# davxy/ark-vrf

Measured on AMD Instinct MI355X. Metric: thin_vrf_batch_verifications_per_sec, higher is better.
Workload: dtype u32x8 (256-bit prime-field Montgomery, integer)

## Files before the change

### ark_vrf_amd/csrc/capi.hip

```cpp
#include "capi_internal.h"
#include "host_sha512.h"
#include "host_shake128.h"
#include "host_sha256.h"
#include "host_sha512_mb.h"
#include <condition_variable>
#include <deque>
#include <mutex>
#include <thread>
#include "proto_dev.h"
#include "vrf_batch.h"
#include "suite_dispatch.h"
#include <chrono>
#include <optional>
#include <stdlib.h>
#include <string.h>

using namespace avrf;

namespace avrf {
double now_us() {
  return std::chrono::duration<double, std::micro>(std::chrono::steady_clock::now().time_since_epoch()).count();
}
}

// ... 156 lines not shown
    HIP_TRY(c->d_misc.ensure(n * 64)); HIP_TRY(c->L->d_scalars.ensure(n * 32)); HIP_TRY(c->L->d_pre.ensure(n * sizeof(te_pre_raw)));
    HIP_TRY(hipMemcpyAsync(c->d_misc.p, bases_mont_xy, n * 64, hipMemcpyHostToDevice, c->stream));
    HIP_TRY(hipMemcpyAsync(c->L->d_scalars.p, scalars_mont, n * 32, hipMemcpyHostToDevice, c->stream));
    HIP_TRY(hipMemsetAsync(c->d_flags.p, 0, 4, c->stream));
    launch_pre_from_affine(c->suite, c->d_misc.as<uint8_t>(), n, c->L->d_pre.as<te_pre_raw>(), c->d_flags.as<uint32_t>(), 0, c->stream, 1);
    launch_scalars_from_mont(c->suite, c->L->d_scalars.as<uint32_t>(), n, c->d_flags.as<uint32_t>(), c->stream);
    HIP_TRY(hipMemcpyAsync(c->h_flags.p, c->d_flags.p, 4, hipMemcpyDeviceToHost, c->stream));
  }
  c->staged_kind = 0;
  if (int e = lane_msm(c, n, &r)) return e;
  if (n && *c->h_flags.as<uint32_t>()) return AVRF_INVALID_DATA;
  uint8_t canon[64];
  finish_point(c, r, canon);
  with_suite(c->suite, [&](auto tag) { using S = typename decltype(tag)::type; using Fq = HostField<typename S::Fq>;
    Fq::store_le(out_mont_xy, Fq::to_mont(Fq::load_le(canon))); Fq::store_le(out_mont_xy + 32, Fq::to_mont(Fq::load_le(canon + 32))); });
  return AVRF_OK;
}

int avrf_g1_msm(avrf_ctx *c, size_t n, const uint8_t *bases_xy, const uint8_t *scalars, uint8_t *out_xy) {
  if (!c || !out_xy || (n && (!bases_xy || !scalars))) return AVRF_ERR_BAD_ARG;
  if (ctx_busy(c)) return AVRF_ERR_BAD_ARG;
  HIP_TRY(hipSetDevice(c->device));
  const int curve = pairing_curve_of(c->suite);
  const size_t fqb = curve == 0 ? 48 : 32;
  for (size_t i = 0; i < n; i++) {
    H256 v; memcpy(v.l, scalars + 32 * i, 32);
    bool ok = curve == 0 ? !HostField<FqBandersnatch>::geq_p(v) : !HostField<FqBabyJubJub>::geq_p(v);
    if (!ok) return AVRF_INVALID_DATA;
  }
  c->staged_kind = 0;
  if (n) {
    HIP_TRY(c->d_misc.ensure(n * 2 * fqb)); HIP_TRY(c->L->d_scalars.ensure(n * 32)); HIP_TRY(c->L->d_pre.ensure(n * 2 * fqb));
    HIP_TRY(hipMemcpyAsync(c->d_misc.p, bases_xy, n * 2 * fqb, hipMemcpyHostToDevice, c->stream));
    HIP_TRY(hipMemcpyAsync(c->L->d_scalars.p, scalars, n * 32, hipMemcpyHostToDevice, c->stream));
    HIP_TRY(hipMemsetAsync(c->d_flags.p, 0, 4, c->stream));
    launch_g1_bases(curve, c->d_misc.as<uint8_t>(), n, c->L->d_pre.as<uint32_t>(), c->d_flags.as<uint32_t>(), c->stream);
    HIP_TRY(hipMemcpyAsync(c->h_flags.p, c->d_flags.p, 4, hipMemcpyDeviceToHost, c->stream));
  }
  if (int e = guarded([&] { return msm_g1_device(curve, c->L->d_pre.as<uint32_t>(), c->L->d_scalars.as<uint32_t>(), n, c->L->ws, c->stream, out_xy) ? (int)AVRF_ERR_BAD_ARG : 0; })) return e;
  if (n && *c->h_flags.as<uint32_t>()) return AVRF_INVALID_DATA;
  return AVRF_OK;
}


}
namespace avrf {
static bool suite_host_weights(int suite) { return with_suite(suite, [&](auto tag) { using S = typename decltype(tag)::type; return (bool)S::HOST_WEIGHTS; }); }
int ctx_stage(avrf_ctx *c, int kind, size_t n, const uint8_t *sks, const uint8_t *pks_xy, const uint8_t *ios_xy,
              const uint32_t *io_counts, const uint8_t *ads, const uint32_t *ad_lens, const uint8_t *proofs, bool wait) {
  if (!c || c->run_phase) return AVRF_ERR_BAD_ARG;
  if (n && (!io_counts || !ad_lens)) return AVRF_ERR_BAD_ARG;
  if (n > 0x0fffffffULL) return AVRF_ERR_BAD_ARG;
  HIP_TRY(hipSetDevice(c->device));
  c->staged_kind = 0; c->n = n; c->tot_io = 0; c->n_terms = 0; c->stage_gen++; c->wire_pending = false;
  if (n == 0) { c->staged_kind = kind; return AVRF_OK; }
  HIP_TRY(c->h_io.ensure((n + 1) * 8));
  uint32_t *io_off = c->h_io.as<uint32_t>(), *ad_off = io_off + (n + 1);
  uint64_t a = 0, b = 0;
  for (size_t j = 0; j < n; j++) { io_off[j] = (uint32_t)a; ad_off[j] = (uint32_t)b; a += io_counts[j]; b += ad_lens[j]; }
  if (a > 0x1fffffffULL || b > 0x7fffffffULL) return AVRF_ERR_BAD_ARG;
  if ((a && !ios_xy) || (b && !ads)) return AVRF_ERR_BAD_ARG;
  io_off[n] = (uint32_t)a; ad_off[n] = (uint32_t)b;
  c->tot_io = (size_t)a;
  HIP_TRY(c->d_io_off.ensure((n + 1) * 4)); HIP_TRY(c->d_ad_off.ensure((n + 1) * 4));
  HIP_TRY(c->d_ios.ensure(a * 128 + 16)); HIP_TRY(c->d_ads.ensure(b + 16));
  HIP_TRY(hipMemcpyAsync(c->d_io_off.p, io_off, (n + 1) * 4, hipMemcpyHostToDevice, c->stream));
  HIP_TRY(hipMemcpyAsync(c->d_ad_off.p, ad_off, (n + 1) * 4, hipMemcpyHostToDevice, c->stream));
  if (a) HIP_TRY(hipMemcpyAsync(c->d_ios.p, ios_xy, a * 128, hipMemcpyHostToDevice, c->stream));
  if (b) HIP_TRY(hipMemcpyAsync(c->d_ads.p, ads, b, hipMemcpyHostToDevice, c->stream));
  const size_t psz = kind == 1 ? 96 : kind == 3 ? 48 : 256;
  if (pks_xy) { HIP_TRY(c->d_pks.ensure(n * 64)); HIP_TRY(hipMemcpyAsync(c->d_pks.p, pks_xy, n * 64, hipMemcpyHostToDevice, c->stream)); }
  if (sks) { HIP_TRY(c->d_sks.ensure(n * 32)); HIP_TRY(hipMemcpyAsync(c->d_sks.p, sks, n * 32, hipMemcpyHostToDevice, c->stream)); }
  if (proofs) {
    HIP_TRY(c->d_proofs.ensure(n * psz)); HIP_TRY(hipMemcpyAsync(c->d_proofs.p, proofs, n * psz, hipMemcpyHostToDevice, c->stream));
    if (kind == 3) { HIP_TRY(hipStreamSynchronize(c->stream)); c->staged_kind = kind; return AVRF_OK; }
    if (suite_host_weights(c->suite)) {
      const size_t rsz = kind == 1 ? 32 : 64, roff = kind == 1 ? 64 : 192;
      c->h_resp.resize(n * rsz);
      for (size_t j = 0; j < n; j++) memcpy(&c->h_resp[rsz * j], proofs + psz * j + roff, rsz);
    }
    c->n_terms = kind == 1 ? 2 * n + 2 * c->tot_io + 1 : 5 * n + 2;
    HIP_TRY(c->d_c.ensure(n * 16)); HIP_TRY(c->h_c.ensure(n * 16));
    HIP_TRY(c->d_z.ensure(kind == 1 ? c->tot_io * 16 + 16 : n * 128));
    if (c->lane_owner) { HIP_TRY(c->L->d_scalars.ensure(c->n_terms * 32)); HIP_TRY(c->L->d_pre.ensure(c->n_terms * sizeof(te_pre_raw))); HIP_TRY(c->L->d_gpart.ensure(((n + 127) / 128) * 64 + 64)); }
  }
  if (wait) HIP_TRY(hipStreamSynchronize(c->stream));
  c->staged_kind = kind;
  return AVRF_OK;
}
int ctx_stage_wire(avrf_ctx *c, int kind, size_t n, const uint8_t *pks, const uint8_t *ios, const uint32_t *io_counts, const uint8_t *ads,
                   const uint32_t *ad_lens, const uint8_t *proofs, int validate, bool wait) {
  if (!c || c->run_phase || (kind != 1 && kind != 2)) return AVRF_ERR_BAD_ARG;
  if (n && (!io_counts || !ad_lens || !proofs || (kind == 1 && !pks))) return AVRF_ERR_BAD_ARG;
  if (n > 0x0fffffffULL) return AVRF_ERR_BAD_ARG;
  HIP_TRY(hipSetDevice(c->device));
  c->staged_kind = 0; c->n = n; c->tot_io = 0; c->n_terms = 0; c->stage_gen++; c->wire_pending = false;
  if (n == 0) { c->staged_kind = kind; return AVRF_OK; }
  HIP_TRY(c->h_io.ensure((n + 1) * 8));
  uint32_t *io_off = c->h_io.as<uint32_t>(), *ad_off = io_off + (n + 1);
  uint64_t a = 0, b = 0;
  for (size_t j = 0; j < n; j++) { io_off[j] = (uint32_t)a; ad_off[j] = (uint32_t)b; a += io_counts[j]; b += ad_lens[j]; }
  if (a > 0x1fffffffULL || b > 0x7fffffffULL) return AVRF_ERR_BAD_ARG;
  if ((a && !ios) || (b && !ads)) return AVRF_ERR_BAD_ARG;
  io_off[n] = (uint32_t)a; ad_off[n] = (uint32_t)b;
  c->tot_io = (size_t)a;
  const size_t L = (size_t)point_len_of(c->suite), ppts = kind == 1 ? 1 : 3, tail = kind == 1 ? 32 : 64, plen = ppts * L + tail, psz = kind == 1 ? 96 : 256;
  const size_t w_pks = kind == 1 ? n * L : 0, w_ios = 2 * (size_t)a * L, w_pr = n * plen;
  HIP_TRY(c->d_io_off.ensure((n + 1) * 4)); HIP_TRY(c->d_ad_off.ensure((n + 1) * 4));
  HIP_TRY(c->d_ios.ensure(a * 128 + 16)); HIP_TRY(c->d_ads.ensure(b + 16)); HIP_TRY(c->d_proofs.ensure(n * psz));
  if (kind == 1) HIP_TRY(c->d_pks.ensure(n * 64));
  HIP_TRY(c->d_misc.ensure(w_pks + w_ios + w_pr + 64)); HIP_TRY(c->d_status.ensure(64));
  uint8_t *dw = c->d_misc.as<uint8_t>();
  HIP_TRY(hipMemcpyAsync(c->d_io_off.p, io_off, (n + 1) * 4, hipMemcpyHostToDevice, c->stream));
  HIP_TRY(hipMemcpyAsync(c->d_ad_off.p, ad_off, (n + 1) * 4, hipMemcpyHostToDevice, c->stream));
  if (b) HIP_TRY(hipMemcpyAsync(c->d_ads.p, ads, b, hipMemcpyHostToDevice, c->stream));
  if (w_pks) HIP_TRY(hipMemcpyAsync(dw, pks, w_pks, hipMemcpyHostToDevice, c->stream));
  if (w_ios) HIP_TRY(hipMemcpyAsync(dw + w_pks, ios, w_ios, hipMemcpyHostToDevice, c->stream));
  HIP_TRY(hipMemcpyAsync(dw + w_pks + w_ios, proofs, w_pr, hipMemcpyHostToDevice, c->stream));
  uint32_t *d_flag = c->d_status.as<uint32_t>(), *h_flag = c->h_flags.as<uint32_t>() + 2;
  HIP_TRY(hipMemsetAsync(d_flag, 0, 4, c->stream));
  if (kind == 1) AVRF_SINGLE(c->suite, decompress_strided(dw, (uint32_t)L, (uint32_t)n, c->d_pks.as<uint8_t>(), 64, validate, d_flag, c->stream));
  AVRF_SINGLE(c->suite, decompress_strided(dw + w_pks, (uint32_t)L, (uint32_t)(2 * a), c->d_ios.as<uint8_t>(), 64, validate, d_flag, c->stream));
  const uint8_t *dpr = dw + w_pks + w_ios;
  for (size_t p = 0; p < ppts; p++)
    AVRF_SINGLE(c->suite, decompress_strided(dpr + L * p, (uint32_t)plen, (uint32_t)n, c->d_proofs.as<uint8_t>() + 64 * p, (uint32_t)psz, validate, d_flag, c->stream));
  HIP_TRY(hipMemcpy2DAsync(c->d_proofs.as<uint8_t>() + 64 * ppts, psz, dpr + L * ppts, plen, tail, n, hipMemcpyDeviceToDevice, c->stream));
  HIP_TRY(hipMemcpyAsync(h_flag, d_flag, 4, hipMemcpyDeviceToHost, c->stream));
  if (suite_host_weights(c->suite)) {
    const size_t rsz = kind == 1 ? 32 : 64, roff = ppts * L;
    c->h_resp.resize(n * rsz);
    for (size_t j = 0; j < n; j++) memcpy(&c->h_resp[rsz * j], proofs + plen * j + roff, rsz);
  }
  c->n_terms = kind == 1 ? 2 * n + 2 * c->tot_io + 1 : 5 * n + 2;
  HIP_TRY(c->d_c.ensure(n * 16)); HIP_TRY(c->h_c.ensure(n * 16));
  HIP_TRY(c->d_z.ensure(kind == 1 ? c->tot_io * 16 + 16 : n * 128));
  if (c->lane_owner) { HIP_TRY(c->L->d_scalars.ensure(c->n_terms * 32)); HIP_TRY(c->L->d_pre.ensure(c->n_terms * sizeof(te_pre_raw))); HIP_TRY(c->L->d_gpart.ensure(((n + 127) / 128) * 64 + 64)); }
  if (!wait) { c->wire_pending = true; c->staged_kind = kind; return AVRF_OK; }
  HIP_TRY(hipStreamSynchronize(c->stream)); HIP_TRY(hipGetLastError());
  if (*h_flag) return AVRF_INVALID_DATA;
  c->staged_kind = kind;
  return AVRF_OK;
}
}
extern "C" {
int avrf_thin_batch_stage_wire(avrf_ctx *c, size_t n, const uint8_t *pks, const uint8_t *ios, const uint32_t *io_counts, const uint8_t *ads,
                               const uint32_t *ad_lens, const uint8_t *proofs, int validate) {
  if (!c || ctx_busy(c)) return AVRF_ERR_BAD_ARG;
  return avrf::ctx_stage_wire(c, 1, n, pks, ios, io_counts, ads, ad_lens, proofs, validate, true);
}
int avrf_pedersen_batch_stage_wire(avrf_ctx *c, size_t n, const uint8_t *ios, const uint32_t *io_counts, const uint8_t *ads,
                                   const uint32_t *ad_lens, const uint8_t *proofs, int validate) {
  if (!c || ctx_busy(c)) return AVRF_ERR_BAD_ARG;
  return avrf::ctx_stage_wire(c, 2, n, nullptr, ios, io_counts, ads, ad_lens, proofs, validate, true);
}

int avrf_thin_batch_stage(avrf_ctx *c, size_t n, const uint8_t *pks_xy, const uint8_t *ios_xy, const uint32_t *io_counts,
                          const uint8_t *ads, const uint32_t *ad_lens, const uint8_t *proofs) {
  if (n && (!pks_xy || !proofs)) return AVRF_ERR_BAD_ARG;
  return ctx_stage(c, 1, n, nullptr, pks_xy, ios_xy, io_counts, ads, ad_lens, proofs, true);
}
int avrf_pedersen_batch_stage(avrf_ctx *c, size_t n, const uint8_t *ios_xy, const uint32_t *io_counts,
                              const uint8_t *ads, const uint32_t *ad_lens, const uint8_t *proofs) {
  if (n && !proofs) return AVRF_ERR_BAD_ARG;
  return ctx_stage(c, 2, n, nullptr, nullptr, ios_xy, io_counts, ads, ad_lens, proofs, true);
}

static void weight_digest_scalar(WeightJob &j) {
  HostSha512 h;
  if (j.msg) { h.update(j.msg, j.msg_len); h.final(j.digest); return; }
  h.update(j.prefix, j.prefix_len);
  uint8_t rec[96]; memset(rec, 0, sizeof rec);
  for (size_t k = 0; k < j.n; k++) { memcpy(rec, j.c16 + 16 * k, 16); memcpy(rec + 32, j.resp + j.rsz * k, j.rsz); h.update(rec, 32 + j.rsz); }
  h.final(j.digest);
}
namespace {
class WeightHashService {
 public:
  static WeightHashService &get() { static WeightHashService s; return s; }
  bool enabled() const { return !workers_.empty(); }
  void run(WeightJob &job) {
    Item it{&job, false};
    std::unique_lock<std::mutex> lk(m_);
    q_.push_back(&it);
    cv_work_.notify_one();
    cv_done_.wait(lk, [&] { return it.done; });
  }
 private:
  struct Item { WeightJob *job; bool done; };
  WeightHashService() {
    int n = 0;
    if (const char *e = getenv("AVRF_HASH_THREADS")) n = atoi(e);
    if (n < 0) n = 0; if (n > 16) n = 16;
    if (!sha512_mb_available()) n = 0;
    for (int i = 0; i < n; i++) workers_.emplace_back([this] { loop(); });
  }
  ~WeightHashService() {
    { std::lock_guard<std::mutex> lk(m_); stop_ = true; }
    cv_work_.notify_all();
    for (auto &t : workers_) t.join();
  }
  void loop() {
    for (;;) {
      Item *take[8]; int cnt = 0;
      {
        std::unique_lock<std::mutex> lk(m_);
        cv_work_.wait(lk, [&] { return stop_ || !q_.empty(); });
        if (stop_) return;
        if (q_.size() == 1) cv_work_.wait_for(lk, std::chrono::microseconds(40), [&] { return stop_ || q_.size() >= 2; });
        if (stop_) return;
        while (cnt < 8 && !q_.empty()) { take[cnt++] = q_.front(); q_.pop_front(); }
      }
      if (cnt == 1) weight_digest_scalar(*take[0]->job);
      else if (cnt > 1) { WeightJob *jobs[8]; for (int i = 0; i < cnt; i++) jobs[i] = take[i]->job; sha512_weights_x8(jobs, cnt); }
      { std::lock_guard<std::mutex> lk(m_); for (int i = 0; i < cnt; i++) take[i]->done = true; }
      cv_done_.notify_all();
    }
  }
  std::mutex m_; std::condition_variable cv_work_, cv_done_; std::deque<Item *> q_; std::vector<std::thread> workers_; bool stop_ = false;
};
// ... 20 lines not shown
  BatchDev b = batch_of(c);
  HIP_TRY(hipMemsetAsync(c->d_flags.p, 0, 4, c->stream));
  validate_staged(c, kind, nullptr);
  const int host_stream = host_stream_kind(c->suite);
  const size_t recsz = kind == 1 ? 64 : 96;
  uint8_t prefix[64]; const size_t pl = batch_prefix(c->suite, prefix);
  if (!host_stream) {
    HIP_TRY(c->d_rec.ensure(n * recsz)); HIP_TRY(c->h_msg.ensure(pl + n * recsz));
    b.records = c->d_rec.as<uint8_t>();
  }
  if (kind == 1) AVRF_BATCH(c->suite, thin_prepare(b, c->d_c.as<uint32_t>(), c->d_z.as<uint32_t>(), c->d_flags.as<uint32_t>(), c->stream));
  else AVRF_BATCH(c->suite, ped_prepare(b, c->d_c.as<uint32_t>(), c->d_z.as<uint8_t>(), c->d_flags.as<uint32_t>(), c->stream));
  if (!host_stream) {
    memcpy(c->h_msg.p, prefix, pl);
    HIP_TRY(hipMemcpyAsync(c->h_msg.as<uint8_t>() + pl, c->d_rec.p, n * recsz, hipMemcpyDeviceToHost, c->stream));
    c->h_msg_len = pl + n * recsz;
  } else HIP_TRY(hipMemcpyAsync(c->h_c.p, c->d_c.p, n * 16, hipMemcpyDeviceToHost, c->stream));
  HIP_TRY(hipMemcpyAsync(c->h_flags.p, c->d_flags.p, 4, hipMemcpyDeviceToHost, c->stream));
  c->run_begin_us = now_us() - c->run_t0;
  c->run_phase = 1;
  return AVRF_OK;
}

int batch_collect(avrf_ctx *c, int kind) {
  if (!c || c->staged_kind != kind || c->run_phase != 1) return AVRF_ERR_BAD_ARG;
  if (c->n && *c->h_flags.as<uint32_t>()) { c->run_phase = 0; return AVRF_INVALID_DATA; }
  if (c->wire_pending) {
    c->wire_pending = false;
    if (c->n && c->h_flags.as<uint32_t>()[2]) { c->run_phase = 0; c->staged_kind = 0; return AVRF_INVALID_DATA; }
  }
  return AVRF_OK;
}

int batch_seed(avrf_ctx *c, int kind, uint8_t digest[64]) {
  const size_t n = c->n;
  memset(digest, 0, 64);
  if (!n) return AVRF_OK;
  const int host_stream = host_stream_kind(c->suite);
  if (host_stream) {
    const uint8_t tag = DS_BATCH_VERIFY;
    const uint8_t *cs = c->h_c.as<uint8_t>();
    const size_t rsz = kind == 1 ? 32 : 64, wsz = kind == 1 ? 16 : 32;
    uint8_t rec[96]; memset(rec, 0, sizeof rec);
    c->h_weights.resize(n * wsz);
    auto run = [&](auto &h) {
      with_suite(c->suite, [&](auto tag_) { using S = typename decltype(tag_)::type; h.update(S::SUITE_ID, S::SUITE_ID_LEN); });
      h.update(&tag, 1);
      for (size_t j = 0; j < n; j++) { memcpy(rec, cs + 16 * j, 16); memcpy(rec + 32, &c->h_resp[rsz * j], rsz); h.update(rec, 32 + rsz); }
      h.squeeze_copy(c->h_weights.data(), n * wsz);
    };
    if (host_stream == 1) { HostShake128 h; run(h); } else { HostSha256 h; run(h); }
    return AVRF_OK;
  }
  WeightJob job; job.prefix = nullptr; job.prefix_len = 0; job.c16 = nullptr; job.resp = nullptr; job.n = n; job.rsz = 0;
  job.msg = c->h_msg.as<uint8_t>(); job.msg_len = c->h_msg_len;
  WeightHashService &svc = WeightHashService::get();
  if (svc.enabled()) svc.run(job); else weight_digest_scalar(job);
  memcpy(digest, job.digest, 64);
  return AVRF_OK;
}

int batch_launch(avrf_ctx *c, int kind, const uint8_t digest[64]) {
  if (!c || c->staged_kind != kind || c->run_phase != 1) return AVRF_ERR_BAD_ARG;
  if (c->n == 0) { c->run_phase = 2; return AVRF_OK; }
  c->run_phase = 0;
  HIP_TRY(hipSetDevice(c->device));
  const size_t n = c->n;
  BatchDev b = batch_of(c);
  if (c->unit_weights) {
    c->h_weights.assign(n * 16, 0);
    for (size_t j = 0; j < n; j++) c->h_weights[16 * j] = 1;
    HIP_TRY(c->d_weights.ensure(n * 16));
    HIP_TRY(hipMemcpyAsync(c->d_weights.p, c->h_weights.data(), n * 16, hipMemcpyHostToDevice, c->stream));
    b.weights = c->d_weights.as<uint8_t>();
  } else if (!host_stream_kind(c->suite)) b.records = c->d_rec.as<uint8_t>();
  else {
    const size_t wsz = kind == 1 ? 16 : 32;
    HIP_TRY(c->d_weights.ensure(n * wsz));
    HIP_TRY(hipMemcpyAsync(c->d_weights.p, c->h_weights.data(), n * wsz, hipMemcpyHostToDevice, c->stream));
    b.weights = c->d_weights.as<uint8_t>();
  }
  Seed64 seed;
  for (int i = 0; i < 8; i++) { uint64_t v; memcpy(&v, digest + 8 * i, 8); seed.w[i] = __builtin_bswap64(v); }
  HIP_TRY(c->L->d_scalars.ensure(c->n_terms * 32)); HIP_TRY(c->L->d_pre.ensure(c->n_terms * sizeof(te_pre_raw))); HIP_TRY(c->L->d_gpart.ensure(((n + 127) / 128) * 64 + 64));
  const double t2 = now_us();
  if (kind == 1) AVRF_BATCH(c->suite, thin_terms(b, seed, 0, c->d_c.as<uint32_t>(), c->d_z.as<uint32_t>(), c->L->d_scalars.as<uint32_t>(),
                                                 c->L->d_pre.as<te_pre_raw>(), c->L->d_gpart.as<uint32_t>(), (uint32_t)c->n_terms, c->stream));
  else AVRF_BATCH(c->suite, ped_terms(b, seed, 0, c->d_c.as<uint32_t>(), c->d_z.as<uint8_t>(), c->L->d_scalars.as<uint32_t>(),
                                      c->L->d_pre.as<te_pre_raw>(), c->L->d_gpart.as<uint32_t>(), (uint32_t)c->n_terms, c->stream));
  const double t3 = now_us();
  if (int e = guarded([&] { return msm_te_enqueue(c->suite, c->L->d_pre.as<te_pre_raw>(), c->L->d_scalars.as<uint32_t>(), c->n_terms, c->L->ws, c->chain(), c->stream) ? (int)AVRF_ERR_BAD_ARG : 0; })) return e;
  c->timing[3] = t3 - t2;
  c->run_msm_us = now_us() - t3;
  c->run_phase = 2;
  return AVRF_OK;
}

int batch_end(avrf_ctx *c, int kind) {
  if (!c || c->staged_kind != kind || c->run_phase != 2) return AVRF_ERR_BAD_ARG;
  c->run_phase = 0;
  if (c->n == 0) return AVRF_OK;
  HIP_TRY(hipSetDevice(c->device));
  const double t3 = now_us();
  HostExt r;
  if (int e = guarded([&] { return msm_te_finish(c->suite, c->L->ws, c->chain(), c->stream, &r) ? (int)AVRF_ERR_BAD_ARG : 0; })) return e;
  double t4 = now_us();
  int st = point_is_identity(c, r) ? AVRF_OK : AVRF_VERIFICATION_FAILURE;
  double t5 = now_us();
  c->timing[4] = c->run_msm_us + (t4 - t3); c->timing[5] = t5 - t4;
  c->timing[0] = c->timing[1] + c->timing[2] + c->timing[3] + c->timing[4] + c->timing[5];
  return st;
}
}
extern "C" {

static int batch_hash(avrf_ctx *c, int kind) {
  if (!c || c->staged_kind != kind || c->run_phase != 1) return AVRF_ERR_BAD_ARG;
  if (c->n == 0) { c->run_phase = 2; return AVRF_OK; }
  HIP_TRY(hipSetDevice(c->device));
  const double tw = now_us();
  if (hipStreamSynchronize(c->stream) != hipSuccess) { c->run_phase = 0; (void)hipGetLastError(); return AVRF_ERR_NO_DEVICE; }
  const double t1 = now_us();
  if (int e = batch_collect(c, kind)) return e;
  uint8_t digest[64];
  if (int e = batch_seed(c, kind, digest)) { c->run_phase = 0; return e; }
  const double t2 = now_us();
  c->timing[1] = c->run_begin_us + (t1 - tw); c->timing[2] = t2 - t1;
  return batch_launch(c, kind, digest);
}

static int batch_run(avrf_ctx *c, int kind) {
  if (int e = batch_begin(c, kind)) return e;
  if (int e = batch_hash(c, kind)) return e;
  return batch_end(c, kind);
}

int avrf_thin_batch_run(avrf_ctx *c) { return batch_run(c, 1); }
int avrf_pedersen_batch_run(avrf_ctx *c) { return batch_run(c, 2); }
static int run_call(avrf_ctx *c, int (*phase)(avrf_ctx *, int)) {
  if (!c) return AVRF_ERR_BAD_ARG;
  if (!c->staged_kind) {
    if (c->run_phase) { (void)hipSetDevice(c->device); (void)hipStreamSynchronize(c->stream); c->run_phase = 0; c->chain().disarm(); }
    return AVRF_ERR_BAD_ARG;
  }
  return phase(c, c->staged_kind);
}
int avrf_batch_run_begin(avrf_ctx *c) { return run_call(c, batch_begin); }
int avrf_batch_run_hash(avrf_ctx *c) { return run_call(c, batch_hash); }
int avrf_batch_run_end(avrf_ctx *c) { return run_call(c, batch_end); }

int avrf_thin_batch_verify(avrf_ctx *c, size_t n, const uint8_t *pks_xy, const uint8_t *ios_xy, const uint32_t *io_counts,
                           const uint8_t *ads, const uint32_t *ad_lens, const uint8_t *proofs) {
  int st = avrf_thin_batch_stage(c, n, pks_xy, ios_xy, io_counts, ads, ad_lens, proofs);
  return st ? st : avrf_thin_batch_run(c);
}
int avrf_pedersen_batch_verify(avrf_ctx *c, size_t n, const uint8_t *ios_xy, const uint32_t *io_counts,
                               const uint8_t *ads, const uint32_t *ad_lens, const uint8_t *proofs) {
  int st = avrf_pedersen_batch_stage(c, n, ios_xy, io_counts, ads, ad_lens, proofs);
  return st ? st : avrf_pedersen_batch_run(c);
}


int avrf_batch_weight_seed(int suite, int pedersen, size_t n, const uint8_t *c16, const uint8_t *resp, uint8_t seed_out[64]) {
  if (suite < 0 || suite >= AVRF_N_SUITES || !seed_out || (n && (!c16 || !resp))) return AVRF_ERR_BAD_ARG;
  if (with_suite(suite, [&](auto tag) { using S = typename decltype(tag)::type; return (bool)S::HOST_WEIGHTS; })) return AVRF_ERR_BAD_ARG;
  HostSha512 h;
  with_suite(suite, [&](auto tag) { using S = typename decltype(tag)::type; h.update(S::SUITE_ID, S::SUITE_ID_LEN); });
  const uint8_t tag = DS_BATCH_VERIFY; h.update(&tag, 1);
  const size_t rsz = pedersen ? 64 : 32;
  uint8_t rec[96]; memset(rec, 0, sizeof rec);
  for (size_t j = 0; j < n; j++) { memcpy(rec, c16 + 16 * j, 16); memcpy(rec + 32, resp + rsz * j, rsz); h.update(rec, 32 + rsz); }
  h.final(seed_out);
  return AVRF_OK;
}

int avrf_batch_weight_seeds_x8(int suite, int pedersen, int count, const size_t *n, const uint8_t *const *c16, const uint8_t *const *resp, uint8_t *seeds_out) {
  if (suite < 0 || suite >= AVRF_N_SUITES || count < 1 || count > 8 || !n || !c16 || !resp || !seeds_out) return AVRF_ERR_BAD_ARG;
  if (with_suite(suite, [&](auto tag) { using S = typename decltype(tag)::type; return (bool)S::HOST_WEIGHTS; })) return AVRF_ERR_BAD_ARG;
  if (!sha512_mb_available()) return AVRF_ERR_NO_DEVICE;
  uint8_t prefix[64]; size_t pl = 0;
  with_suite(suite, [&](auto tag) { using S = typename decltype(tag)::type; memcpy(prefix, S::SUITE_ID, S::SUITE_ID_LEN); pl = S::SUITE_ID_LEN; });
  prefix[pl++] = DS_BATCH_VERIFY;
  WeightJob jobs[8]; WeightJob *pj[8];
  for (int i = 0; i < count; i++) {
    if (n[i] && (!c16[i] || !resp[i])) return AVRF_ERR_BAD_ARG;
    jobs[i].prefix = prefix; jobs[i].prefix_len = pl; jobs[i].c16 = c16[i]; jobs[i].resp = resp[i]; jobs[i].n = n[i]; jobs[i].rsz = pedersen ? 64 : 32; pj[i] = &jobs[i];
  }
  sha512_weights_x8(pj, count);
  for (int i = 0; i < count; i++) memcpy(seeds_out + 64 * i, jobs[i].digest, 64);
  return AVRF_OK;
}

int avrf_sha512_x8(int count, const uint8_t *const *msgs, const size_t *lens, uint8_t *digests_out) {
  if (count < 1 || count > 8 || !msgs || !lens || !digests_out) return AVRF_ERR_BAD_ARG;
  if (!sha512_mb_available()) return AVRF_ERR_NO_DEVICE;
  static const uint8_t empty = 0;
  WeightJob jobs[8]; WeightJob *pj[8];
  for (int i = 0; i < count; i++) {
    if (lens[i] && !msgs[i]) return AVRF_ERR_BAD_ARG;
    jobs[i].msg = lens[i] ? msgs[i] : &empty; jobs[i].msg_len = lens[i]; pj[i] = &jobs[i];
  }
  sha512_weights_x8(pj, count);
  for (int i = 0; i < count; i++) memcpy(digests_out + 64 * i, jobs[i].digest, 64);
  return AVRF_OK;
}

int avrf_sha512_x16(int count, const uint8_t *const *msgs, const size_t *lens, uint8_t *digests_out) {
  if (count < 1 || count > 16 || !msgs || !lens || !digests_out) return AVRF_ERR_BAD_ARG;
  if (!sha512_mb16_available()) return AVRF_ERR_NO_DEVICE;
  static const uint8_t empty = 0;
  WeightJob jobs[16]; WeightJob *pj[16];
  for (int i = 0; i < count; i++) {
    if (lens[i] && !msgs[i]) return AVRF_ERR_BAD_ARG;
    jobs[i].msg = lens[i] ? msgs[i] : &empty; jobs[i].msg_len = lens[i]; pj[i] = &jobs[i];
  }
  sha512_weights_x16(pj, count);
  for (int i = 0; i < count; i++) memcpy(digests_out + 64 * i, jobs[i].digest, 64);
  return AVRF_OK;
}

int avrf_thin_batch_challenges(avrf_ctx *c, uint8_t *c_out) {
  if (!c || c->staged_kind != 1 || (c->n && !c_out)) return AVRF_ERR_BAD_ARG;
  if (ctx_busy(c)) return AVRF_ERR_BAD_ARG;
  if (c->n == 0) return AVRF_OK;
  HIP_TRY(hipSetDevice(c->device));
// ... 113 lines not shown

static int sync_stream(avrf_ctx *c) {
  HIP_TRY(hipStreamSynchronize(c->stream)); HIP_TRY(hipGetLastError());
  return AVRF_OK;
}

static bool wave_shape(const avrf_ctx *c, size_t n, const uint32_t *io_counts) {
  if (!n || n > (size_t)AVRF_WAVE_ITEMS_MAX || c->tot_io != n) return false;
  static const bool off = getenv("AVRF_NO_WAVE_ITEMS") != nullptr;
  if (off) return false;
  for (size_t j = 0; j < n; j++) if (io_counts[j] != 1) return false;
  return true;
}

using Route = std::optional<int>;
static bool one_as_msm() { static const bool on = getenv("AVRF_NO_ONE_AS_MSM") == nullptr; return on; }

static Route prove_one_as_msm(avrf_ctx *c, bool have_pk, bool tiny, uint8_t *proofs_out) {
  if (c->tot_io >= 1000) return {};
  const size_t nt = 1 + c->tot_io, plen = tiny ? 48 : 96, sb = AVRF_SINGLE(c->suite, prove_state_bytes());
  HIP_TRY(c->h_c.ensure(64));
  if (!have_pk) { if (int fs = ensure_fixed(c)) return fs; }
  HIP_TRY(c->L->d_scalars.ensure(nt * 32)); HIP_TRY(c->L->d_pre.ensure(nt * sizeof(te_pre_raw))); HIP_TRY(c->d_misc.ensure(sb + 64)); HIP_TRY(c->d_out.ensure(plen));
  BatchDev b = batch_of(c);
  if (!have_pk) b.pks_xy = nullptr;
  uint8_t *d_state = c->d_misc.as<uint8_t>();
  AVRF_SINGLE(c->suite, thin_prove_begin(b, c->L->d_scalars.as<uint32_t>(), c->L->d_pre.as<te_pre_raw>(), d_state, c->stream, tiny));
  HostExt r;
  if (int e = lane_msm(c, nt, &r)) return e;
  uint8_t *rxy = c->h_c.as<uint8_t>();
  finish_point(c, r, rxy);
  HIP_TRY(hipMemcpyAsync(d_state + sb, rxy, 64, hipMemcpyHostToDevice, c->stream));
  AVRF_SINGLE(c->suite, thin_prove_end(b, d_state, d_state + sb, c->d_out.as<uint8_t>(), c->d_flags.as<uint32_t>(), c->stream, tiny));
  HIP_TRY(hipMemcpyAsync(proofs_out, c->d_out.p, plen, hipMemcpyDeviceToHost, c->stream));
  return read_flags(c);
}

static Route prove_ped_one_as_msm(avrf_ctx *c, bool have_pk, uint8_t *proofs_out, uint8_t *blindings_out) {
  if (c->tot_io > 1000) return {};
  if (!have_pk) { if (int fs = ensure_fixed(c)) return fs; }
  const size_t m = c->tot_io, nt = 2 + m, sb = AVRF_SINGLE(c->suite, ped_state_bytes()), wb = (m * 32 + 63) / 64 * 64 + 64;
  HIP_TRY(c->L->d_scalars.ensure(2 * nt * 32)); HIP_TRY(c->L->d_pre.ensure(nt * sizeof(te_pre_raw)));
  HIP_TRY(c->d_misc.ensure(sb + wb + 192 + 32)); HIP_TRY(c->d_out.ensure(256)); HIP_TRY(c->h_c.ensure(192));
  BatchDev b = batch_of(c);
  if (!have_pk) b.pks_xy = nullptr;
  uint8_t *d_state = c->d_misc.as<uint8_t>(), *d_pts = d_state + sb + wb, *d_blind = d_pts + 192;
  uint32_t *d_wts = reinterpret_cast<uint32_t *>(d_state + sb);
  uint32_t *d_sc = c->L->d_scalars.as<uint32_t>(); te_pre_raw *d_pre = c->L->d_pre.as<te_pre_raw>();
  AVRF_SINGLE(c->suite, ped_prove_begin(b, d_sc, d_pre, d_state, d_wts, c->stream));
  HostExt r[2];
  if (int e = lane_msm(c, 2, &r[0])) return e;
  uint8_t *pts = c->h_c.as<uint8_t>();
  finish_point(c, r[0], pts);
  HIP_TRY(hipMemcpyAsync(d_pts, pts, 64, hipMemcpyHostToDevice, c->stream));
  AVRF_SINGLE(c->suite, ped_prove_mid(b, d_sc, d_pre, d_state, d_wts, d_pts, c->stream));
  if (int e = lane_msm_vectors(c, nt, 2, r)) return e;
  finish_point(c, r[0], pts + 64); finish_point(c, r[1], pts + 128);
  HIP_TRY(hipMemcpyAsync(d_pts + 64, pts + 64, 128, hipMemcpyHostToDevice, c->stream));
  AVRF_SINGLE(c->suite, ped_prove_end(b, d_state, d_pts, c->d_out.as<uint8_t>(), blindings_out ? d_blind : nullptr, c->d_flags.as<uint32_t>(), c->stream));
  HIP_TRY(hipMemcpyAsync(proofs_out, c->d_out.p, 256, hipMemcpyDeviceToHost, c->stream));
  if (blindings_out) HIP_TRY(hipMemcpyAsync(blindings_out, d_blind, 32, hipMemcpyDeviceToHost, c->stream));
  return read_flags(c);
}

static Route verify_one_as_msm(avrf_ctx *c, int32_t *status_out) {
  if (!c->n_terms || c->n_terms > 2048) return {};
  uint8_t zero[64] = {0};
  c->unit_weights = true;
  int st = batch_begin(c, 1);
  if (st == AVRF_OK) st = batch_launch(c, 1, zero);
  if (st == AVRF_OK) st = batch_end(c, 1);
  c->unit_weights = false;
  if (st != AVRF_OK && st != AVRF_VERIFICATION_FAILURE) { c->run_phase = 0; return st; }
  status_out[0] = *c->h_flags.as<uint32_t>() ? AVRF_INVALID_DATA : st;
  return AVRF_OK;
}

static Route verify_ped_one_as_msm(avrf_ctx *c, int32_t *status_out) {
  if (!c->n_terms || c->n_terms > 2048) return {};
  int st = batch_begin(c, 2);
  c->run_phase = 0;
  if (st != AVRF_OK) return st;
  const size_t nt = c->n_terms;
  HIP_TRY(c->L->d_scalars.ensure(2 * nt * 32)); HIP_TRY(c->L->d_pre.ensure(nt * sizeof(te_pre_raw))); HIP_TRY(c->L->d_gpart.ensure(2 * 64 + 64));
  c->h_weights.assign(64, 0); c->h_weights[0] = 1; c->h_weights[32 + 16] = 1;
  HIP_TRY(c->d_weights.ensure(64));
  HIP_TRY(hipMemcpyAsync(c->d_weights.p, c->h_weights.data(), 64, hipMemcpyHostToDevice, c->stream));
  BatchDev b = batch_of(c);
  Seed64 seed; for (int i = 0; i < 8; i++) seed.w[i] = 0;
  for (int v = 0; v < 2; v++) {
    b.weights = c->d_weights.as<uint8_t>() + 32 * v;
    AVRF_BATCH(c->suite, ped_terms(b, seed, 0, c->d_c.as<uint32_t>(), c->d_z.as<uint8_t>(), c->L->d_scalars.as<uint32_t>() + (size_t)v * nt * 8,
                                   c->L->d_pre.as<te_pre_raw>(), c->L->d_gpart.as<uint32_t>(), (uint32_t)nt, c->stream));
  }
  HostExt r[2];
  if (int e = lane_msm_vectors(c, nt, 2, r)) return e;
  status_out[0] = *c->h_flags.as<uint32_t>() ? AVRF_INVALID_DATA : (point_is_identity(c, r[0]) && point_is_identity(c, r[1])) ? AVRF_OK : AVRF_VERIFICATION_FAILURE;
  return AVRF_OK;
}

struct ItemCall {
  int kind;
  bool prover;
  size_t psz;
  uint8_t *proofs_out;
  uint8_t *blindings_out;
  int32_t *status_out;
};

template <class One, class Wave, class Lane>
static int item_call(avrf_ctx *c, const ItemCall &k, size_t n, const uint8_t *sks, const uint8_t *pks_xy, const uint8_t *ios_xy,
                     const uint32_t *io_counts, const uint8_t *ads, const uint32_t *ad_lens, const uint8_t *proofs, One one, Wave wave, Lane lane) {
  int st = ctx_stage(c, k.kind, n, sks, pks_xy, ios_xy, io_counts, ads, ad_lens, proofs, k.kind == 3);
  if (st || !n) return st;
  if (k.prover) {
    c->staged_kind = 0;
    HIP_TRY(c->d_out.ensure(n * k.psz));
    if (k.kind == 2) HIP_TRY(c->d_misc.ensure(n * 32));
  } else HIP_TRY(c->d_status.ensure(n * 4));
  if (k.prover || k.kind == 3) HIP_TRY(hipMemsetAsync(c->d_flags.p, 0, 4, c->stream));
  auto finish = [&](bool wave_statuses) -> int {
    if (!k.prover) {
      validate_staged(c, k.kind, c->d_status.as<int32_t>());
      HIP_TRY(hipMemcpyAsync(k.status_out, c->d_status.p, n * 4, hipMemcpyDeviceToHost, c->stream));
      return sync_stream(c);
    }
    HIP_TRY(hipMemcpyAsync(k.proofs_out, c->d_out.p, n * k.psz, hipMemcpyDeviceToHost, c->stream));
    if (k.blindings_out) HIP_TRY(hipMemcpyAsync(k.blindings_out, c->d_misc.p, n * 32, hipMemcpyDeviceToHost, c->stream));
    if (wave_statuses) HIP_TRY(hipMemcpyAsync(c->h_c.p, c->d_status.p, n * 4, hipMemcpyDeviceToHost, c->stream));
    return read_flags(c);
  };
  auto routes = [&]() -> int {
    if (n == 1 && one_as_msm()) { if (Route r = one()) return *r; }
    if ((!k.prover || pks_xy) && wave_shape(c, n, io_counts)) {
      if (k.prover && k.kind == 2) { if (int fs = ensure_fixed(c)) return fs; }
      if (k.prover) { HIP_TRY(c->d_status.ensure(n * 4)); HIP_TRY(c->h_c.ensure(n * 4)); }
      if (wave(batch_of(c))) {
        const int ws = finish(true);
        if (ws < 0) return ws;
        const int32_t *h_status = k.prover ? c->h_c.as<int32_t>() : k.status_out;
        bool fallback = false;
        for (size_t j = 0; j < n; j++) fallback |= h_status[j] == AVRF_WAVE_FALLBACK;
        if (!fallback) return ws;
        if (k.prover) HIP_TRY(hipMemsetAsync(c->d_flags.p, 0, 4, c->stream));
      }
    }
    if (int e = per_item_chunks(c, !k.prover || pks_xy, lane)) return e;
    return finish(false);
  };
  const double t0 = now_us();
  st = routes();
  c->timing[0] = now_us() - t0;
  if (k.kind == 3 && st == AVRF_OK) c->staged_kind = 0;
  return st;
}

template <class F> static int pointwise(avrf_ctx *c, size_t n, bool args_ok, F body) {
  if (!c || (n && !args_ok) || ctx_busy(c)) return AVRF_ERR_BAD_ARG;
  if (!n) return AVRF_OK;
  if (n > 0x7fffffffULL) return AVRF_ERR_BAD_ARG;
  HIP_TRY(hipSetDevice(c->device));
  c->staged_kind = 0;
  return body();
}
extern "C" {

static int thin_or_tiny_prove(avrf_ctx *c, bool tiny, size_t n, const uint8_t *sks, const uint8_t *pks_xy, const uint8_t *ios_xy,
// ... 156 lines not shown
```

### ark_vrf_amd/csrc/capi_internal.h

```cpp
#pragma once
#include "../../include/avrf.h"
#include "host_te.h"
#include "msm.h"
#include <hip/hip_runtime.h>
#include <stdio.h>
#include <new>
#include <vector>

#define HIP_TRY(x) do { hipError_t e_ = (x); if (e_ != hipSuccess) { fprintf(stderr, "avrf: HIP error %s at %s:%d\n", hipGetErrorString(e_), __FILE__, __LINE__); return AVRF_ERR_NO_DEVICE; } } while (0)

namespace avrf {

template <bool PINNED> struct StageBuf : OwnedMem<PINNED> {
  hipError_t ensure(size_t bytes) {
    if (bytes <= this->cap && this->p) return hipSuccess;
    return this->reset(PINNED ? bytes + 256 : bytes + bytes / 8 + 256);
  }
};
using DevBuf = StageBuf<false>;
using PinBuf = StageBuf<true>;

template <class F> int guarded(F f) {
  try { return f(); }
  catch (const avrf::HipFailure &e) { fprintf(stderr, "avrf: HIP error %s at %s:%d\n", hipGetErrorString(e.err), e.file, e.line); return AVRF_ERR_NO_DEVICE; }
  catch (const std::bad_alloc &) { return AVRF_ERR_NO_DEVICE; }
}

struct LaneStream {
  hipStream_t stream = nullptr;
  LaneStream() = default;
  LaneStream(const LaneStream &) = delete;
  LaneStream &operator=(const LaneStream &) = delete;
  ~LaneStream() { if (stream) (void)hipStreamDestroy(stream); }
};
struct Lane : LaneStream {
  int queued = 0;
  MsmWorkspace ws;
  DevBuf d_scalars, d_pre, d_gpart;
};

}

struct avrf_ctx {
  int suite = 0, device = 0;
  hipStream_t stream = nullptr;
  avrf::Lane own; avrf::Lane *L = &own;
  avrf::MsmChain *pend = nullptr;
  avrf::MsmChain &chain() const { return pend ? *pend : L->ws.own; }
  bool lane_owner = true;
  int validate = 0;
  bool wire_pending = false;
  uint64_t stage_gen = 0, chal_gen = 0;
  int staged_kind = 0;
  size_t n = 0, tot_io = 0, n_terms = 0;
  avrf::DevBuf d_pks, d_ios, d_io_off, d_ads, d_ad_off, d_proofs, d_sks;
  std::vector<uint8_t> h_resp;
  avrf::DevBuf d_rec; avrf::PinBuf h_msg;
  size_t h_msg_len = 0;
  std::vector<uint8_t> h_weights; avrf::DevBuf d_weights;
  avrf::DevBuf d_c, d_z, d_flags, d_misc, d_out, d_status;
  avrf::DevBuf d_tabs;
  avrf::DevBuf d_fixed; bool fixed_ready = false;
  avrf::PinBuf h_c, h_flags, h_io;
  double timing[8] = {0, 0, 0, 0, 0, 0, 0, 0};
  int run_phase = 0;
  bool unit_weights = false;
  double run_t0 = 0, run_begin_us = 0, run_msm_us = 0;
  ~avrf_ctx() { (void)hipSetDevice(device); if (own.stream) (void)hipStreamSynchronize(own.stream); }
};

namespace avrf {
int ctx_create(int suite, int device, bool lane_owner, avrf_ctx **out);
int ctx_stage(avrf_ctx *c, int kind, size_t n, const uint8_t *sks, const uint8_t *pks_xy, const uint8_t *ios_xy, const uint32_t *io_counts,
              const uint8_t *ads, const uint32_t *ad_lens, const uint8_t *proofs, bool wait);
int ctx_stage_wire(avrf_ctx *c, int kind, size_t n, const uint8_t *pks, const uint8_t *ios, const uint32_t *io_counts, const uint8_t *ads,
                   const uint32_t *ad_lens, const uint8_t *proofs, int validate, bool wait);
int batch_begin(avrf_ctx *c, int kind);
int batch_collect(avrf_ctx *c, int kind);
bool batch_host_weights(const avrf_ctx *c);
int batch_seed(avrf_ctx *c, int kind, uint8_t digest[64]);
int batch_launch(avrf_ctx *c, int kind, const uint8_t digest[64]);
int batch_end(avrf_ctx *c, int kind);
double now_us();
}
```

### ark_vrf_amd/csrc/msm.h

```cpp
#pragma once
#include <hip/hip_runtime.h>
#include <stddef.h>
#include <stdint.h>
#include "host_te.h"

namespace avrf {

struct te_pre_raw { uint32_t w[24]; };
struct te_ext_raw { uint32_t w[32]; };

struct HipFailure { hipError_t err; const char *file; int line; };

template <bool PINNED> struct OwnedMem {
  void *p = nullptr; size_t cap = 0;
  OwnedMem() = default;
  explicit OwnedMem(size_t bytes) { ensure(bytes); }
  OwnedMem(const OwnedMem &) = delete;
  OwnedMem &operator=(const OwnedMem &) = delete;
  OwnedMem(OwnedMem &&o) noexcept : p(o.p), cap(o.cap) { o.p = nullptr; o.cap = 0; }
  OwnedMem &operator=(OwnedMem &&o) noexcept { if (this != &o) { (void)release(); p = o.p; cap = o.cap; o.p = nullptr; o.cap = 0; } return *this; }
  ~OwnedMem() { (void)release(); }
  hipError_t reset(size_t bytes) {
    if (hipError_t e = release()) return e;
    if (hipError_t e = PINNED ? hipHostMalloc(&p, bytes) : hipMalloc(&p, bytes)) { p = nullptr; return e; }
    cap = bytes;
    return hipSuccess;
  }
  void ensure(size_t bytes) { if (bytes > cap) if (hipError_t e = reset(bytes)) throw HipFailure{e, __FILE__, __LINE__}; }
  hipError_t release() { hipError_t e = !p ? hipSuccess : PINNED ? hipHostFree(p) : hipFree(p); p = nullptr; cap = 0; return e; }
  template <class T = uint32_t> T *as() const { return (T *)p; }
  explicit operator bool() const { return p != nullptr; }
};
using DevMem = OwnedMem<false>;
using PinMem = OwnedMem<true>;
struct DevEvent {
  hipEvent_t e = nullptr;
  DevEvent() = default;
  DevEvent(const DevEvent &) = delete;
  DevEvent &operator=(const DevEvent &) = delete;
  DevEvent(DevEvent &&o) noexcept : e(o.e) { o.e = nullptr; }
  DevEvent &operator=(DevEvent &&o) noexcept { if (this != &o) { destroy(); e = o.e; o.e = nullptr; } return *this; }
  ~DevEvent() { destroy(); }
  hipError_t create(unsigned flags = hipEventDefault) { destroy(); return hipEventCreateWithFlags(&e, flags); }
  void destroy() { if (e) (void)hipEventDestroy(e); e = nullptr; }
  operator hipEvent_t() const { return e; }
};

struct MsmPlan {
  int c;
  int nwin;
  int nb;
  int lpb;
};
MsmPlan msm_plan(size_t n, int scalar_bits);

struct MsmChain {
  PinMem bits_host, plan_host;
  DevEvent ev0, ev1;
  MsmPlan plan = {0, 0, 0, 0}; int ret = 0;
  int wsum_lg = 4;
  size_t n = 0;
  bool armed = false;
  void ensure(size_t bytes);
  void disarm() { armed = false; }
  void release() { *this = MsmChain(); }
};

struct MsmWorkspace {
  DevMem keys;
  DevMem sorted;
  DevMem hist;
  DevMem cnts;
  DevMem offsets;
  DevMem win_tot;
  DevMem lane_base;
  DevMem heavy;
  DevMem plan_dev;
  DevMem buckets;
  DevMem rc;
  DevMem part;
  DevMem bits;
  MsmChain own;
  bool owns(const MsmChain &rec) const { return &rec == &own; }
  double accum_ms_total = 0; uint64_t accum_launches = 0; float accum_ms_last = 0;
  MsmPlan last_plan = {0, 0, 0, 0};
  void ensure(size_t n, const MsmPlan &p, size_t acc_bytes, size_t batch, size_t lanes_max, size_t part_bytes = 0);
  void release() { *this = MsmWorkspace(); }
};

int msm_te_device(int suite, const te_pre_raw *d_pre, const uint32_t *d_scalars, size_t n,
                  MsmWorkspace &ws, hipStream_t stream, HostExt *out);
int msm_te_enqueue(int suite, const te_pre_raw *d_pre, const uint32_t *d_scalars, size_t n, MsmWorkspace &ws, MsmChain &rec, hipStream_t stream);
int msm_te_finish(int suite, MsmWorkspace &ws, MsmChain &rec, hipStream_t stream, HostExt *out);
int msm_te_small_vectors(int suite, const te_pre_raw *d_pre, const uint32_t *d_scalars, size_t n, size_t n_vectors, MsmWorkspace &ws, hipStream_t stream,
                         HostExt *out);
bool msm_te_pending_supported(int suite);

int msm_g1_device(int curve, const uint32_t *d_bases, const uint32_t *d_scalars, size_t n, MsmWorkspace &ws, hipStream_t stream, uint8_t *out_xy,
                  size_t batch = 1, size_t scalar_stride = 0);
void build_g1_table(int curve, const uint32_t *d_bases, size_t n, int c, int nwin, uint32_t *d_table, hipStream_t stream);
int msm_g1_fixed_device(int curve, const uint32_t *d_table, int table_c, size_t table_stride, const uint32_t *d_scalars, size_t n,
                        size_t scalar_stride, MsmWorkspace &ws, hipStream_t stream, uint8_t *out_xy, size_t batch,
                        const uint32_t *d_base_idx = nullptr, int scalars_mont = 0);
struct G1DirectTable {
  uint32_t *d = nullptr;
  int curve = 0, c = 0, rows = 0;
  size_t n = 0;
  uint64_t off[32] = {};
  uint32_t mult[32] = {};
  uint64_t points = 0, bytes = 0;
};
size_t g1_direct_table_shape(int curve, size_t n, int c, G1DirectTable *t);
void build_g1_direct_table(int curve, const uint32_t *d_bases, size_t n, int c, G1DirectTable *t, hipStream_t stream);
void free_g1_direct_table(G1DirectTable *t);
int msm_g1_direct_device(const G1DirectTable &t, const uint32_t *d_scalars, size_t n, size_t scalar_stride, MsmWorkspace &ws, hipStream_t stream,
                         uint8_t *out_xy, size_t batch, int scalars_mont = 0, const uint32_t *d_base_idx = nullptr);
void launch_g1_decompress(int curve, const uint8_t *d_comp, size_t n, uint8_t *d_out_xy, uint8_t *d_ok, hipStream_t stream);
void launch_g1_bases(int curve, const uint8_t *d_xy, size_t n, uint32_t *d_out, uint32_t *d_flag, hipStream_t stream);
void launch_g1_subgroup_check(int curve, const uint32_t *d_bases, size_t n, uint32_t *d_flag, hipStream_t stream, int32_t *d_rec_status = nullptr,
                              uint32_t ppr = 1);
void launch_g1_lincomb(int curve, const uint32_t *d_bases, const uint32_t *d_scalars, size_t n_items, uint32_t tpi, uint32_t split, uint32_t *d_out,
                       hipStream_t stream, bool glv_split_scalars = false);
void g1_glv_split_bls(uint64_t k[4]);

void launch_pre_from_affine(int suite, const uint8_t *d_xy, size_t n, te_pre_raw *d_pre, uint32_t *d_flag,
                            int check_curve, hipStream_t stream, int mont_in = 0);
void launch_scalars_from_mont(int suite, uint32_t *d_scalars, size_t n, uint32_t *d_flag, hipStream_t stream);

}
```

### ark_vrf_amd/csrc/msm.hip

```cpp
#include "msm.h"
#include "host_pool.h"
#include "curves.h"
#include "suite_dispatch.h"
#include "te_quad.h"
#include "host_g1.h"
#include <stdio.h>
#include <stdlib.h>
#include <string.h>
#include <mutex>
#include <vector>

namespace avrf {

#define HIP_CHECK(x) do { hipError_t e_ = (x); if (e_ != hipSuccess) throw HipFailure{e_, __FILE__, __LINE__}; } while (0)


template <class S>
__global__ void __launch_bounds__(256) k_pre_from_affine(const uint8_t *__restrict__ xy, uint32_t n, te_pre *__restrict__ out,
                                  uint32_t *__restrict__ flag, int check_curve, int mont_in) {
  using Fq = typename S::Fq;
  uint32_t i = blockIdx.x * blockDim.x + threadIdx.x;
  if (i >= n) return;
  fp x = fp_load_le(xy + 64 * (size_t)i), y = fp_load_le(xy + 64 * (size_t)i + 32);
  uint32_t f = 0;
  if (ge_p<Fq>(x) || ge_p<Fq>(y)) f |= 1;
  fp xm = mont_in ? x : fp_to_mont<Fq>(x), ym = mont_in ? y : fp_to_mont<Fq>(y);
  if (check_curve && !te_on_curve<S>(xm, ym)) f |= 2;
  store_pre(out + i, te_make_pre<S>(xm, ym));
  if (f) atomicOr(flag, f);
}

void launch_pre_from_affine(int suite, const uint8_t *d_xy, size_t n, te_pre_raw *d_pre, uint32_t *d_flag,
                            int check_curve, hipStream_t stream, int mont_in) {
  if (!n) return;
  dim3 g((unsigned)((n + 255) / 256)), b(256);
  with_suite(suite, [&](auto tag) { using S = typename decltype(tag)::type;
    hipLaunchKernelGGL(k_pre_from_affine<S>, g, b, 0, stream, d_xy, (uint32_t)n, (te_pre *)d_pre, d_flag, check_curve, mont_in); });
}
template <class S>
__global__ void __launch_bounds__(256) k_scalars_from_mont(uint32_t *__restrict__ sc, uint32_t n, uint32_t *__restrict__ flag) {
  using Fr = typename S::Fr;
  uint32_t i = blockIdx.x * blockDim.x + threadIdx.x;
  if (i >= n) return;
  fp k = load_fp(sc + 8 * (size_t)i);
  if (ge_p<Fr>(k)) atomicOr(flag, 4u);
  store_fp(sc + 8 * (size_t)i, fp_from_mont<Fr>(k));
}
void launch_scalars_from_mont(int suite, uint32_t *d_scalars, size_t n, uint32_t *d_flag, hipStream_t stream) {
  if (!n) return;
  with_suite(suite, [&](auto tag) { using S = typename decltype(tag)::type;
    hipLaunchKernelGGL(k_scalars_from_mont<S>, dim3((unsigned)((n + 255) / 256)), dim3(256), 0, stream, d_scalars, (uint32_t)n, d_flag); });
}


__global__ void __launch_bounds__(256) k_digits(const uint32_t *__restrict__ scalars, uint32_t n, uint32_t stride, int c, int nwin, uint16_t *__restrict__ keys, int mont) {
  uint32_t i = blockIdx.x * blockDim.x + threadIdx.x;
  if (i >= n) return;
  const uint32_t bat = blockIdx.y;
  keys += (size_t)bat * nwin * n;
  uint32_t s[9];
  const uint4 *p = reinterpret_cast<const uint4 *>(scalars + 8 * ((size_t)bat * stride + i));
  uint4 a = p[0], b = p[1];
  s[0] = a.x; s[1] = a.y; s[2] = a.z; s[3] = a.w; s[4] = b.x; s[5] = b.y; s[6] = b.z; s[7] = b.w; s[8] = 0;
  if (mont) {
    fp v;
#pragma unroll
    for (int k = 0; k < 8; k++) v.v[k] = s[k];
    v = mont == 1 ? fp_from_mont<FqBandersnatch>(v) : fp_from_mont<FqBabyJubJub>(v);
#pragma unroll
    for (int k = 0; k < 8; k++) s[k] = v.v[k];
  }
  const uint32_t nb = 1u << (c - 1), mask = (1u << c) - 1;
  uint32_t carry = 0;
  for (int w = 0; w < nwin; w++) {
    int bit = w * c;
    uint32_t v = 0;
    if (bit < 256) {
      int li = bit >> 5, sh = bit & 31;
      uint64_t two = (uint64_t)s[li] | ((uint64_t)s[li + 1] << 32);
      v = (uint32_t)(two >> sh) & mask;
    }
    v += carry;
    uint32_t key;
    if (v > nb) { key = ((1u << c) - v) | 0x8000u; carry = 1; }
    else { key = v; carry = 0; }
    keys[(size_t)w * n + i] = (uint16_t)key;
  }
}


__global__ void __launch_bounds__(256)
k_hist(const uint16_t *__restrict__ keys, uint32_t n, uint32_t tile_len, int c, uint32_t *__restrict__ H) {
  extern __shared__ uint32_t lds[];
  const uint32_t nb = 1u << (c - 1), tile = blockIdx.x, w = blockIdx.y, ntiles = gridDim.x;
  for (uint32_t b = threadIdx.x; b < nb; b += blockDim.x) lds[b] = 0;
  __syncthreads();
  uint32_t lo = tile * tile_len, hi = lo + tile_len; if (hi > n) hi = n;
  const uint16_t *kw = keys + (size_t)w * n;
  for (uint32_t i = lo + threadIdx.x; i < hi; i += blockDim.x) {
    uint32_t b = kw[i] & 0x7fffu;
    if (b) atomicAdd(&lds[b - 1], 1u);
  }
  __syncthreads();
  uint32_t *out = H + ((size_t)w * ntiles + tile) * nb;
  for (uint32_t b = threadIdx.x; b < nb; b += blockDim.x) out[b] = lds[b];
}

__global__ void __launch_bounds__(256)
k_scan_tiles(uint32_t *__restrict__ H, uint32_t ntiles, int c, uint32_t *__restrict__ cnts) {
  const uint32_t nb = 1u << (c - 1), w = blockIdx.y, b = blockIdx.x * 256 + threadIdx.x;
  if (b >= nb) return;
  uint32_t *Hb = H + (size_t)w * ntiles * nb + b;
  uint32_t run = 0, k = 0;
  for (; k + 8 <= ntiles; k += 8) {
    uint32_t v[8];
#pragma unroll
    for (int j = 0; j < 8; j++) v[j] = Hb[(size_t)(k + j) * nb];
#pragma unroll
    for (int j = 0; j < 8; j++) { Hb[(size_t)(k + j) * nb] = run; run += v[j]; }
  }
  for (; k < ntiles; k++) { const uint32_t v = Hb[(size_t)k * nb]; Hb[(size_t)k * nb] = run; run += v; }
  cnts[(size_t)w * nb + b] = run;
}
__global__ void __launch_bounds__(1024)
k_scan_offs(const uint32_t *__restrict__ cnts, uint32_t n, int c, uint32_t *__restrict__ offs, uint32_t *__restrict__ win_tot) {
  __shared__ uint32_t part[1024];
  const uint32_t nb = 1u << (c - 1), w = blockIdx.x, t = threadIdx.x;
  const uint32_t bpt = (nb + 1023) / 1024;
  uint32_t b0 = t * bpt, b1 = b0 + bpt; if (b1 > nb) b1 = nb; if (b0 > nb) b0 = nb;
  uint32_t sum = 0;
  for (uint32_t b = b0; b < b1; b++) sum += cnts[(size_t)w * nb + b];
  part[t] = sum;
  __syncthreads();
  for (uint32_t off = 1; off < 1024; off <<= 1) {
    uint32_t v = (t >= off) ? part[t - off] : 0;
    __syncthreads();
    part[t] += v;
    __syncthreads();
  }
  if (t == 1023) win_tot[w] = part[1023];
  uint32_t run = part[t] - sum + w * n;
  for (uint32_t b = b0; b < b1; b++) { offs[(size_t)w * nb + b] = run; run += cnts[(size_t)w * nb + b]; }
}

__global__ void __launch_bounds__(1024)
k_plan(const uint32_t *__restrict__ win_tot, uint32_t vwin, uint32_t lanes_target, uint32_t per_min, uint32_t *__restrict__ lane_base,
       uint32_t *__restrict__ plan) {
  __shared__ uint64_t red[1024];
  __shared__ uint32_t sc[1024];
  __shared__ uint32_t carry_s;
  const uint32_t t = threadIdx.x;
  uint64_t s = 0;
  for (uint32_t v = t; v < vwin; v += 1024) s += win_tot[v];
  red[t] = s;
  __syncthreads();
  for (uint32_t off = 512; off >= 1; off >>= 1) { if (t < off) red[t] += red[t + off]; __syncthreads(); }
  const uint64_t total = red[0];
  if (lanes_target > 8 * vwin) lanes_target -= vwin;
  uint64_t per64 = (total + lanes_target - 1) / lanes_target;
  if (per64 < per_min) per64 = per_min;
  const uint32_t per = (uint32_t)per64;
  if (t == 0) carry_s = 0;
  __syncthreads();
  for (uint32_t base = 0; base < vwin; base += 1024) {
    const uint32_t v = base + t;
    const uint32_t mine = v < vwin ? (win_tot[v] + per - 1) / per : 0;
    sc[t] = mine;
    __syncthreads();
    for (uint32_t off = 1; off < 1024; off <<= 1) {
      uint32_t x = (t >= off) ? sc[t - off] : 0;
      __syncthreads();
      sc[t] += x;
      __syncthreads();
    }
    if (v < vwin) lane_base[v] = carry_s + sc[t] - mine;
    __syncthreads();
    if (t == 1023) carry_s += sc[1023];
    __syncthreads();
  }
  if (t == 0) { lane_base[vwin] = carry_s; plan[0] = per; plan[1] = carry_s; plan[2] = 0; }
}

__global__ void __launch_bounds__(256)
k_scatter(const uint16_t *__restrict__ keys, uint32_t n, uint32_t tile_len, int c, const uint32_t *__restrict__ H,
          const uint32_t *__restrict__ offs, uint32_t *__restrict__ sorted, uint32_t remap_n, uint32_t remap_stride,
          const uint32_t *__restrict__ bidx, uint32_t ntiles, uint32_t vwin) {
  extern __shared__ uint32_t lds[];
  const uint32_t nb = 1u << (c - 1);
  const uint32_t xcd = blockIdx.x & 7u, k = blockIdx.x >> 3, tile = k % ntiles, w = xcd + 8u * (k / ntiles);
  if (w >= vwin) return;
  const uint32_t *Hin = H + ((size_t)w * ntiles + tile) * nb;
  for (uint32_t b = threadIdx.x; b < nb; b += blockDim.x) lds[b] = offs[(size_t)w * nb + b] + Hin[b];
  __syncthreads();
  uint32_t lo = tile * tile_len, hi = lo + tile_len; if (hi > n) hi = n;
  const uint16_t *kw = keys + (size_t)w * n;
  for (uint32_t i = lo + threadIdx.x; i < hi; i += blockDim.x) {
    uint32_t key = kw[i], b = key & 0x7fffu;
    if (b) {
      uint32_t pos = atomicAdd(&lds[b - 1], 1u);
      uint32_t idx = i;
      if (remap_n) {
        uint32_t j = i % remap_n;
        idx = (i / remap_n) * remap_stride + (bidx ? bidx[(size_t)w * remap_n + j] : j);
      }
      sorted[pos] = idx | ((key & 0x8000u) << 16);
    }
  }
}

template <class CV> __device__ __noinline__ void cv_add_nf(typename CV::acc_t *r, const typename CV::acc_t *a, const typename CV::acc_t *b) { *r = CV::add(*a, *b); }
template <class CV> __device__ __noinline__ void cv_dbl_nf(typename CV::acc_t *r, const typename CV::acc_t *a) { *r = CV::dbl(*a); }
template <class CV> AVRF_DI typename CV::acc_t cv_add(const typename CV::acc_t &a, const typename CV::acc_t &b) {
  if constexpr (CV::INLINE_REDUCE_OPS) return CV::add(a, b);
  else { typename CV::acc_t r; cv_add_nf<CV>(&r, &a, &b); return r; }
}
template <class CV> AVRF_DI typename CV::acc_t cv_dbl(const typename CV::acc_t &a) {
  if constexpr (CV::INLINE_REDUCE_OPS) return CV::dbl(a);
  else { typename CV::acc_t r; cv_dbl_nf<CV>(&r, &a); return r; }
}



template <class CV>
__global__ void __launch_bounds__(256, CV::MIN_WAVES)
k_accumulate(const uint32_t *__restrict__ bases, const uint32_t *__restrict__ sorted,
             const uint32_t *__restrict__ offs, const uint32_t *__restrict__ win_tot, const uint32_t *__restrict__ lane_base,
             const uint32_t *__restrict__ plan, uint32_t vwin, uint32_t nb, uint32_t n, uint32_t *__restrict__ part) {
  using AC = typename CV::accum;
  using acc_t = typename AC::acc_t; using base_t = typename CV::base_t;
  const uint32_t t = blockIdx.x * blockDim.x + threadIdx.x;
  const uint32_t per = plan[0];
  if (t >= plan[1]) return;
  uint32_t lo = 0, hi = vwin;
  while (hi - lo > 1) { uint32_t mid = (lo + hi) >> 1; if (lane_base[mid] <= t) lo = mid; else hi = mid; }
  const uint32_t v = lo;
  const uint32_t wbeg = v * n, wend = wbeg + win_tot[v];
  const uint32_t e0 = wbeg + (t - lane_base[v]) * per;
  uint32_t e1 = e0 + per; if (e1 > wend) e1 = wend;
  const uint32_t *ow = offs + (size_t)v * nb;
  lo = 0; hi = nb;
  while (hi - lo > 1) { uint32_t mid = (lo + hi) >> 1; if (ow[mid] <= e0) lo = mid; else hi = mid; }
  uint32_t b = lo;
  uint32_t nxt = (b + 1 < nb) ? ow[b + 1] : 0xffffffffu;
  const size_t slot0 = (size_t)t + (size_t)v * nb;
  acc_t acc;
  {
    extern __shared__ uint32_t acc_lds[];
    constexpr int BW = CV::BASE_WORDS, CH = BW / 4;
    uint32_t *wbuf = acc_lds + (threadIdx.x >> 6) * (2 * BW * 64);
    const uint32_t lane = threadIdx.x & 63;
    auto issue = [&](uint32_t ix, uint32_t slot) {
      const uint32_t *src = bases + (size_t)(ix & 0x7fffffffu) * BW;
#pragma unroll
      for (int c = 0; c < CH; c++)
        __builtin_amdgcn_global_load_lds((const __attribute__((address_space(1))) void *)(src + 4 * c),
                                         (__attribute__((address_space(3))) void *)(wbuf + slot * (BW * 64) + c * 256), 16, 0, 0);
    };
    auto fetch = [&](uint32_t slot) {
      uint32_t w[BW];
#pragma unroll
      for (int c = 0; c < CH; c++) {
        const uint4 v = *reinterpret_cast<const uint4 *>(wbuf + slot * (BW * 64) + c * 256 + lane * 4);
        w[4 * c] = v.x; w[4 * c + 1] = v.y; w[4 * c + 2] = v.z; w[4 * c + 3] = v.w;
      }
      return CV::base_from_words(w);
    };
    const uint32_t cnt = e1 - e0;
    if constexpr (!CV::PREFETCH) acc = AC::identity();
    uint32_t idx = cnt ? sorted[e0] : 0u;
    uint32_t idx1 = cnt > 1 ? sorted[e0 + 1] : 0u;
    if (cnt) issue(idx, 0);
    for (uint32_t k = 0; k < cnt; k++) {
      const uint32_t i = e0 + k, cidx = idx;
      asm volatile("s_waitcnt vmcnt(0) lgkmcnt(0)" ::: "memory");
      const base_t cur = fetch(k & 1);
      idx = idx1;
      if (k + 1 < cnt) issue(idx, (k + 1) & 1);
      if (k + 2 < cnt) idx1 = sorted[i + 2];
      if constexpr (CV::PREFETCH) {
        if (k == 0) { acc = AC::from_base(cur, (cidx & 0x80000000u) != 0); continue; }
      }
      if (i >= nxt) {
        AC::store_part(part + (slot0 + b) * AC::PART_WORDS, acc);
        acc = AC::identity();
        do { b++; nxt = (b + 1 < nb) ? ow[b + 1] : 0xffffffffu; } while (i >= nxt);
      }
      acc = AC::madd(acc, cur, (cidx & 0x80000000u) != 0);
    }
  }
  AC::store_part(part + (slot0 + b) * AC::PART_WORDS, acc);
}

template <class T> struct type_tag { using type = T; };
template <class CV> AVRF_DI typename CV::acc_t wave_sum(typename CV::acc_t acc);

constexpr uint32_t HEAVY_PARTIALS = 12;
template <class CV>
__global__ void __launch_bounds__(256, CV::RED_WAVES)
k_bucket_sum(const uint32_t *__restrict__ offs, const uint32_t *__restrict__ cnts, const uint32_t *__restrict__ lane_base,
             uint32_t *__restrict__ plan, uint32_t nslots, uint32_t nb, uint32_t n, const uint32_t *__restrict__ part,
             uint32_t *__restrict__ buckets, uint32_t *__restrict__ heavy) {
  using acc_t = typename CV::acc_t;
  const uint32_t slot = blockIdx.x * blockDim.x + threadIdx.x;
  if (slot >= nslots) return;
  const uint32_t per = plan[0];
  const uint32_t cnt = cnts[slot];
  if (!cnt) { if (!CV::ZERO_IS_IDENTITY) CV::store_acc(buckets + (size_t)slot * CV::ACC_WORDS, CV::identity()); return; }
  const uint32_t v = slot / nb, rel = offs[slot] - v * n;
  const uint32_t lf = rel / per, ll = (rel + cnt - 1) / per, np = ll - lf + 1;
  if (np > HEAVY_PARTIALS) { heavy[atomicAdd(&plan[2], 1u)] = slot; return; }
  const size_t p0 = (size_t)lane_base[v] + lf + slot;
  using AC = typename CV::accum;
  acc_t acc = AC::load_part(part + p0 * AC::PART_WORDS);
#pragma unroll 1
  for (uint32_t k = 1; k < np; k++) acc = cv_add<CV>(acc, AC::load_part(part + (p0 + k) * AC::PART_WORDS));
  CV::store_acc(buckets + (size_t)slot * CV::ACC_WORDS, acc);
}

template <class CV>
__global__ void __launch_bounds__(256, CV::RED_WAVES)
k_heavy_sum(const uint32_t *__restrict__ offs, const uint32_t *__restrict__ cnts, const uint32_t *__restrict__ lane_base,
            const uint32_t *__restrict__ plan, uint32_t nb, uint32_t n, const uint32_t *__restrict__ part,
            uint32_t *__restrict__ buckets, const uint32_t *__restrict__ heavy) {
  using acc_t = typename CV::acc_t;
  extern __shared__ uint32_t lds[];
  const uint32_t per = plan[0], nheavy = plan[2], t = threadIdx.x, lane = t & 63, wv = t >> 6;
  for (uint32_t h = blockIdx.x; h < nheavy; h += gridDim.x) {
    const uint32_t slot = heavy[h], cnt = cnts[slot];
    const uint32_t v = slot / nb, rel = offs[slot] - v * n;
    const uint32_t lf = rel / per, ll = (rel + cnt - 1) / per, np = ll - lf + 1;
    const size_t p0 = (size_t)lane_base[v] + lf + slot;
    if constexpr (CV::QUAD) { q_heavy_sum<typename CV::suite>(part, p0, np, buckets + (size_t)slot * CV::ACC_WORDS, lds); continue; }
    acc_t a = CV::identity();
#pragma unroll 1
    for (uint32_t k = t; k < np; k += 256) a = cv_add<CV>(a, CV::accum::load_part(part + (p0 + k) * CV::accum::PART_WORDS));
    a = wave_sum<CV>(a);
    if (lane == 0) CV::store_acc(lds + wv * CV::ACC_WORDS, a);
    __syncthreads();
    if (t == 0) {
#pragma unroll 1
      for (uint32_t w = 1; w < 4; w++) a = cv_add<CV>(a, CV::load_acc(lds + w * CV::ACC_WORDS));
      CV::store_acc(buckets + (size_t)slot * CV::ACC_WORDS, a);
    }
    __syncthreads();
  }
}


template <class CV> AVRF_DI typename CV::acc_t wave_sum(typename CV::acc_t acc) {
#pragma unroll 1
  for (int off = 32; off >= 1; off >>= 1) acc = cv_add<CV>(acc, CV::shfl_down(acc, off));
  return acc;
}

template <class CV>
__global__ void __launch_bounds__(256)
k_rowcol(const uint32_t *__restrict__ buckets, int c, int h, uint32_t total_waves, uint32_t *__restrict__ rc) {
  const uint32_t nb = 1u << (c - 1), NC = 1u << h, NR = nb >> h;
  const uint32_t gw = (blockIdx.x * blockDim.x + threadIdx.x) >> 6, lane = threadIdx.x & 63;
  if (gw >= total_waves) return;
  const uint32_t tasks = NR + NC, w = gw / tasks, task = gw - w * tasks;
  const uint32_t *B = buckets + (size_t)w * nb * CV::ACC_WORDS;
  typename CV::acc_t acc = CV::identity();
  if (task < NR) {
    for (uint32_t lo = lane; lo < NC; lo += 64) { uint32_t b = task * NC + lo; if (b >= 1) acc = CV::add(acc, CV::load_acc(B + (size_t)(b - 1) * CV::ACC_WORDS)); }
  } else {
    uint32_t lo = task - NR;
    for (uint32_t hi = lane; hi < NR; hi += 64) { uint32_t b = hi * NC + lo; if (b >= 1) acc = CV::add(acc, CV::load_acc(B + (size_t)(b - 1) * CV::ACC_WORDS)); }
  }
  acc = wave_sum<CV>(acc);
  if (lane == 0) CV::store_acc(rc + (size_t)gw * CV::ACC_WORDS, acc);
}

template <class CV>
__global__ void __launch_bounds__(256)
k_bits(const uint32_t *__restrict__ buckets, const uint32_t *__restrict__ rc, int c, int h, uint32_t total_waves, uint32_t *__restrict__ out) {
  const uint32_t nb = 1u << (c - 1), NC = 1u << h, NR = nb >> h;
  const uint32_t gw = (blockIdx.x * blockDim.x + threadIdx.x) >> 6, lane = threadIdx.x & 63;
  if (gw >= total_waves) return;
  const uint32_t w = gw / c, k = gw - w * c;
  const uint32_t *RC = rc + (size_t)w * (NR + NC) * CV::ACC_WORDS;
  typename CV::acc_t acc = CV::identity();
  if ((int)k == c - 1) { if (lane == 0) acc = CV::load_acc(buckets + ((size_t)w * nb + (nb - 1)) * CV::ACC_WORDS); }
  else if ((int)k < h) { for (uint32_t lo = lane; lo < NC; lo += 64) if ((lo >> k) & 1) acc = CV::add(acc, CV::load_acc(RC + (size_t)(NR + lo) * CV::ACC_WORDS)); }
  else { uint32_t kk = k - h; for (uint32_t hi = lane; hi < NR; hi += 64) if ((hi >> kk) & 1) acc = CV::add(acc, CV::load_acc(RC + (size_t)hi * CV::ACC_WORDS)); }
  acc = wave_sum<CV>(acc);
  if (lane == 0) CV::store_acc(out + (size_t)gw * CV::ACC_WORDS, acc);
}

template <class CV>
__global__ void __launch_bounds__(128)
k_bits_direct(const uint32_t *__restrict__ buckets, int c, uint32_t total, uint32_t *__restrict__ out) {
  const uint32_t t = blockIdx.x * blockDim.x + threadIdx.x;
  if (t >= total) return;
  const uint32_t nb = 1u << (c - 1), w = t / c, k = t - w * c;
  const uint32_t *B = buckets + (size_t)w * nb * CV::ACC_WORDS;
  typename CV::acc_t acc = CV::identity();
  if ((int)k == c - 1) acc = CV::load_acc(B + (size_t)(nb - 1) * CV::ACC_WORDS);
  else for (uint32_t m = 0; m < (nb >> 1); m++) {
    uint32_t b = ((m >> k) << (k + 1)) | (1u << k) | (m & ((1u << k) - 1));
    acc = CV::add(acc, CV::load_acc(B + (size_t)(b - 1) * CV::ACC_WORDS));
  }
  CV::store_acc(out + (size_t)t * CV::ACC_WORDS, acc);
}

template <class CV>
__global__ void __launch_bounds__(64)
k_horner(const uint32_t *__restrict__ bits, uint32_t nbits, uint32_t batch, uint32_t *__restrict__ out) {
  uint32_t b = blockIdx.x * blockDim.x + threadIdx.x;
  if (b >= batch) return;
  const uint32_t *T = bits + (size_t)b * nbits * CV::ACC_WORDS;
  typename CV::acc_t acc = CV::identity();
  for (int i = (int)nbits - 1; i >= 0; i--) {
    acc = CV::dbl(acc);
    acc = CV::add(acc, CV::load_acc(T + (size_t)i * CV::ACC_WORDS));
  }
  CV::store_acc(out + (size_t)b * CV::ACC_WORDS, acc);
}

template <class CV>
__global__ void __launch_bounds__(256, CV::RED_WAVES)
k_wsum(const uint32_t *__restrict__ buckets, uint32_t nb, uint32_t nsets, uint32_t lps_log, uint32_t *__restrict__ out) {
  using acc_t = typename CV::acc_t;
  const uint32_t t = blockIdx.x * blockDim.x + threadIdx.x;
  const uint32_t lps = 1u << lps_log, set = t >> lps_log, g = t & (lps - 1), m = nb >> lps_log;
  const bool live = set < nsets;
  acc_t S = CV::identity(), W = CV::identity();
  if (live) {
// ... 90 lines not shown
static uint32_t tile_len_for(size_t n, size_t vwin) { return vwin >= 64 && msm_env().tile ? (uint32_t)msm_env().tile : 8192u; }

MsmPlan msm_plan(size_t n, int scalar_bits) {
  MsmPlan p;
  int lg = 0; while (((size_t)1 << (lg + 1)) <= n) lg++;
  int c = lg >= 16 ? lg - 5 : lg - 3;
  if (c < 4) c = 4; if (c > 15) c = 15;
  p.c = msm_env().c ? msm_env().c : c; p.lpb = 0;
  p.nb = 1 << (p.c - 1);
  p.nwin = (scalar_bits + 1 + p.c - 1) / p.c;
  return p;
}


struct AccShape { size_t lanes; unsigned lds; };
template <class CV> static AccShape accumulate_shape() {
  static AccShape cache[64] = {};
  static std::mutex mu;
  int dev = 0; HIP_CHECK(hipGetDevice(&dev));
  if (dev < 0 || dev >= 64) dev = 0;
  std::lock_guard<std::mutex> lk(mu);
  if (!cache[dev].lanes) {
    int cus = 0, blocks = 0, lds_cu = 0, lds_blk = 0;
    HIP_CHECK(hipDeviceGetAttribute(&cus, hipDeviceAttributeMultiprocessorCount, dev));
    HIP_CHECK(hipOccupancyMaxActiveBlocksPerMultiprocessor(&blocks, k_accumulate<CV>, 256, 0));
    if (blocks < 1) blocks = 1;
    if (hipDeviceGetAttribute(&lds_cu, hipDeviceAttributeMaxSharedMemoryPerMultiprocessor, dev) != hipSuccess || lds_cu <= 0) { (void)hipGetLastError(); lds_cu = 0; }
    if (hipDeviceGetAttribute(&lds_blk, hipDeviceAttributeMaxSharedMemoryPerBlock, dev) != hipSuccess || lds_blk <= 0) { (void)hipGetLastError(); lds_blk = 64 * 1024; }
    {
      hipDeviceProp_t prop;
      if (hipGetDeviceProperties(&prop, dev) == hipSuccess && !strncmp(prop.gcnArchName, "gfx950", 6)) {
        if (lds_cu < 160 * 1024) lds_cu = 160 * 1024;
        if (lds_blk < 160 * 1024) lds_blk = 160 * 1024;
      } else (void)hipGetLastError();
    }
    int cap = CV::MAX_WAVES;
    if (msm_env().occ) cap = msm_env().occ;
    unsigned lds = 0;
    if (cap >= 1 && cap < blocks && lds_cu > 0) {
      const unsigned slice = (unsigned)(lds_cu / (cap + 1) + 1024);
      if ((size_t)slice * cap <= (size_t)lds_cu && slice <= (unsigned)lds_blk) {
        blocks = cap; lds = slice;
        if (lds > 48 * 1024) HIP_CHECK(hipFuncSetAttribute((const void *)k_accumulate<CV>, hipFuncAttributeMaxDynamicSharedMemorySize, (int)lds));
      }
    }
    {
      const unsigned need = 4u * 2u * CV::BASE_WORDS * 64u * 4u;
      if (lds < need) lds = need;
      if (lds > 48 * 1024) HIP_CHECK(hipFuncSetAttribute((const void *)k_accumulate<CV>, hipFuncAttributeMaxDynamicSharedMemorySize, (int)lds));
      int blk2 = 0;
      HIP_CHECK(hipOccupancyMaxActiveBlocksPerMultiprocessor(&blk2, k_accumulate<CV>, 256, lds));
      if (blk2 >= 1 && blk2 < blocks) blocks = blk2;
    }
    cache[dev] = AccShape{(size_t)cus * blocks * 256, lds};
  }
  return cache[dev];
}
template <class CV> static size_t accumulate_lanes() { return accumulate_shape<CV>().lanes; }

static bool msm_poison() { static const bool on = getenv("AVRF_MSM_POISON") != nullptr; return on; }
static void poison(void *p, size_t bytes, int which) {
  if (!msm_poison() || !p) return;
  if (const char *e = getenv("AVRF_MSM_POISON_SKIP")) { if (atoi(e) == which) return; }
  HIP_CHECK(hipMemset(p, 0xA5, bytes)); if (!getenv("AVRF_MSM_POISON_NOSYNC")) HIP_CHECK(hipDeviceSynchronize());
}
static void ws_buf(DevMem &m, size_t bytes, int which) {
  if (bytes <= m.cap) return;
  m.ensure(bytes);
  poison(m.p, bytes, which);
}

void MsmWorkspace::ensure(size_t n, const MsmPlan &p, size_t acc_bytes, size_t batch, size_t lanes_max, size_t part_bytes) {
  const size_t vwin = (size_t)p.nwin * batch;
  const size_t nbk = vwin * p.nb, nbits = vwin * p.c;
  const size_t need_n = vwin * n;
  const size_t ntiles = (n + tile_len_for(n, vwin) - 1) / tile_len_for(n, vwin);
  ws_buf(keys, need_n * 2 + 16, 1); ws_buf(sorted, need_n * 4 + 16, 2);
  ws_buf(hist, nbk * ntiles * 4 + 64, 3);
  ws_buf(cnts, nbk * 4, 4); ws_buf(offsets, nbk * 4, 5); ws_buf(heavy, nbk * 4, 6);
  ws_buf(win_tot, (vwin + 64) * 4, 7); ws_buf(lane_base, (vwin + 64) * 4, 8);
  plan_dev.ensure(64);
  ws_buf(buckets, nbk * acc_bytes, 9); ws_buf(rc, nbk * acc_bytes, 10);
  ws_buf(part, (lanes_max + nbk + 64) * (part_bytes ? part_bytes : acc_bytes) + 64, 11);
  ws_buf(bits, nbits * acc_bytes, 12); own.ensure(nbits * acc_bytes);
}

void MsmChain::ensure(size_t bytes) {
  if (!plan_host) { plan_host.ensure(64); plan_host.as()[0] = plan_host.as()[1] = 0; }
  if (!ev0) { HIP_CHECK(ev0.create()); HIP_CHECK(ev1.create()); }
  bits_host.ensure(bytes);
}

static void msm_collect(MsmWorkspace &ws, MsmChain &rec, hipStream_t stream) {
  if (ws.owns(rec)) { HIP_CHECK(hipStreamSynchronize(stream)); HIP_CHECK(hipGetLastError()); }
  HIP_CHECK(hipEventElapsedTime(&ws.accum_ms_last, rec.ev0, rec.ev1));
  rec.plan.lpb = (int)rec.plan_host.as()[0];
  ws.accum_ms_total += ws.accum_ms_last; ws.accum_launches++; ws.last_plan = rec.plan;
}

constexpr size_t MSM_TINY_TERMS = 2048, MSM_TINY_VECTORS = 32;
template <class CV>
__global__ void __launch_bounds__(256)
k_msm_tiny_bits(const uint32_t *__restrict__ bases, const uint32_t *__restrict__ scalars, uint32_t n, uint32_t stride, uint32_t *__restrict__ out) {
  extern __shared__ uint32_t lds[];
  const uint32_t p = blockIdx.x, v = blockIdx.y, t = threadIdx.x, T = blockDim.x, lane = t & 63, wv = t >> 6, nw = T >> 6;
  typename CV::acc_t acc = CV::identity();
  bool first = true;
#pragma unroll 1
  for (uint32_t k = t; k < n; k += T) {
    if (!((scalars[8 * ((size_t)v * stride + k) + (p >> 5)] >> (p & 31)) & 1u)) continue;
    const typename CV::base_t q = CV::load_base(bases + (size_t)k * CV::BASE_WORDS);
    acc = first ? CV::from_base(q, false) : CV::madd(acc, q, false);
    first = false;
  }
  uint32_t span = 1; while (span < n && span < 64) span <<= 1;
#pragma unroll 1
  for (uint32_t off = span >> 1; off >= 1; off >>= 1) acc = cv_add<CV>(acc, CV::shfl_down(acc, (int)off));
  if (nw > 1) {
    if (lane == 0) CV::store_acc(lds + wv * CV::ACC_WORDS, acc);
    __syncthreads();
    if (wv == 0) {
      acc = lane < nw ? CV::load_acc(lds + lane * CV::ACC_WORDS) : CV::identity();
#pragma unroll 1
      for (uint32_t off = nw >> 1; off >= 1; off >>= 1) acc = cv_add<CV>(acc, CV::shfl_down(acc, (int)off));
    }
  }
  if (t == 0) CV::store_acc(out + ((size_t)v * gridDim.x + p) * CV::ACC_WORDS, acc);
}

struct MsmLaunch {
  size_t batch = 1;
  int table_c = 0; size_t table_stride = 0;
  size_t scalar_stride = 0;
  const uint32_t *d_base_idx = nullptr;
  bool defer = false;
  int scalars_mont = 0;
};

template <class CV>
static int msm_device(const uint32_t *d_bases, const uint32_t *d_scalars, size_t n_in, int scalar_bits, MsmWorkspace &ws, MsmChain &rec, hipStream_t stream,
                      const MsmLaunch &o = MsmLaunch()) {
  const size_t batch = o.batch, scalar_stride = o.scalar_stride ? o.scalar_stride : n_in;
  const int table_c = o.table_c, scalars_mont = o.scalars_mont;
  const uint32_t *const d_base_idx = o.d_base_idx;
  MsmPlan p = msm_plan(n_in, scalar_bits);
  auto finish = [&]() { if (!o.defer) msm_collect(ws, rec, stream); };
  if (n_in <= MSM_TINY_TERMS && batch <= (CV::FIXED_TABLE ? (size_t)7 : MSM_TINY_VECTORS) && !table_c && !d_base_idx && !scalars_mont && msm_env().tiny) {
    p.c = 1; p.nwin = scalar_bits; p.nb = 1; p.lpb = 0;
    const size_t acc_b = (size_t)CV::ACC_WORDS * 4, nbits = (size_t)scalar_bits;
    ws.ensure(n_in, p, acc_b, batch, 256);
    rec.ensure(batch * nbits * acc_b); rec.plan_host.as()[0] = 0; rec.plan = p;
    HIP_CHECK(hipEventRecord(rec.ev0, stream));
    unsigned threads = 64; while (threads < n_in && threads < 256) threads <<= 1;
    hipLaunchKernelGGL(k_msm_tiny_bits<CV>, dim3((unsigned)nbits, (unsigned)batch), dim3(threads), (threads / 64) * acc_b, stream, d_bases, d_scalars, (uint32_t)n_in,
                       (uint32_t)scalar_stride, ws.bits.as());
    HIP_CHECK(hipEventRecord(rec.ev1, stream));
    HIP_CHECK(hipMemcpyAsync(rec.bits_host.p, ws.bits.p, batch * nbits * acc_b, hipMemcpyDeviceToHost, stream));
    finish();
    return (int)nbits;
  }
  const size_t lanes_target = accumulate_lanes<CV>();
  size_t n = n_in;
  uint32_t remap_n = 0, remap_stride = 0;
  dim3 b256(256);
  int dig_nwin = p.nwin;
  if (table_c) {
    dig_nwin = (scalar_bits + 1 + table_c - 1) / table_c;
    p.c = table_c; p.nb = 1 << (table_c - 1); p.nwin = 1;
    n = n_in * (size_t)dig_nwin;
    remap_n = (uint32_t)n_in; remap_stride = (uint32_t)o.table_stride;
  }
  using RV = typename CV::red;
  const bool red = CV::FIXED_TABLE && table_c != 0;
  const size_t acc_bytes = (size_t)(red ? (int)RV::ACC_WORDS : (int)CV::ACC_WORDS) * 4;
  const uint32_t vwin = (uint32_t)(p.nwin * batch);
  const size_t lanes_max = lanes_target + vwin + 256;
  if ((size_t)vwin * n >= 0xffff0000ull) throw HipFailure{hipErrorInvalidValue, __FILE__, __LINE__};
  ws.ensure(n, p, acc_bytes, batch, lanes_max, (size_t)CV::accum::PART_WORDS * 4);
  const uint32_t nbk = vwin * p.nb;
  const uint32_t tile_len = tile_len_for(n, vwin), ntiles = (uint32_t)((n + tile_len - 1) / tile_len);
  const size_t lds_bytes = (size_t)p.nb * 4;
  hipLaunchKernelGGL(k_digits, dim3((unsigned)((n_in + 255) / 256), (unsigned)batch), b256, 0, stream, d_scalars, (uint32_t)n_in, (uint32_t)scalar_stride,
                     p.c, dig_nwin, ws.keys.as<uint16_t>(), scalars_mont);
  hipLaunchKernelGGL(k_hist, dim3(ntiles, vwin), b256, lds_bytes, stream, ws.keys.as<uint16_t>(), (uint32_t)n, tile_len, p.c, ws.hist.as());
  hipLaunchKernelGGL(k_scan_tiles, dim3((unsigned)((p.nb + 255) / 256), vwin), b256, 0, stream, ws.hist.as(), ntiles, p.c, ws.cnts.as());
  hipLaunchKernelGGL(k_scan_offs, dim3(vwin), dim3(1024), 0, stream, ws.cnts.as(), (uint32_t)n, p.c, ws.offsets.as(), ws.win_tot.as());
  hipLaunchKernelGGL(k_plan, dim3(1), dim3(1024), 0, stream, ws.win_tot.as(), vwin, (uint32_t)lanes_target, (uint32_t)msm_env().per_min,
                     ws.lane_base.as(), ws.plan_dev.as());
  hipLaunchKernelGGL(k_scatter, dim3(8u * ((vwin + 7u) / 8u) * ntiles), b256, lds_bytes, stream, ws.keys.as<uint16_t>(), (uint32_t)n, tile_len, p.c, ws.hist.as(),
                     ws.offsets.as(), ws.sorted.as(), remap_n, remap_stride, d_base_idx, ntiles, vwin);
  rec.ensure((size_t)vwin * 3 * acc_bytes);
  if (CV::ZERO_IS_IDENTITY) HIP_CHECK(hipMemsetAsync(ws.buckets.p, 0, (size_t)nbk * acc_bytes, stream));
  HIP_CHECK(hipEventRecord(rec.ev0, stream));
  hipLaunchKernelGGL(k_accumulate<CV>, dim3((unsigned)((lanes_max + 255) / 256)), b256, accumulate_shape<CV>().lds, stream, d_bases, ws.sorted.as(),
                     ws.offsets.as(), ws.win_tot.as(), ws.lane_base.as(), ws.plan_dev.as(), vwin, (uint32_t)p.nb, (uint32_t)n, ws.part.as());
  HIP_CHECK(hipEventRecord(rec.ev1, stream));
  auto bucket_sums = [&](auto tag) {
    using BV = typename decltype(tag)::type;
    hipLaunchKernelGGL(k_bucket_sum<BV>, dim3((nbk + 255) / 256), b256, 0, stream, ws.offsets.as(), ws.cnts.as(), ws.lane_base.as(), ws.plan_dev.as(), nbk,
                       (uint32_t)p.nb, (uint32_t)n, ws.part.as(), ws.buckets.as(), ws.heavy.as());
    hipLaunchKernelGGL(k_heavy_sum<BV>, dim3(nbk < 1024 ? nbk : 1024), b256, 4 * acc_bytes, stream, ws.offsets.as(), ws.cnts.as(), ws.lane_base.as(),
                       ws.plan_dev.as(), (uint32_t)p.nb, (uint32_t)n, ws.part.as(), ws.buckets.as(), ws.heavy.as());
  };
  if (red) bucket_sums(type_tag<RV>{}); else bucket_sums(type_tag<CV>{});
  HIP_CHECK(hipMemcpyAsync(rec.plan_host.p, ws.plan_dev.p, 8, hipMemcpyDeviceToHost, stream));
  rec.plan = p;
  if constexpr (CV::WINDOW_SUMS) if (batch == 1 && msm_env().window_sums) {
    const uint32_t nb = (uint32_t)p.nb;
    const uint32_t wpw = nb >= 256 ? 16u : 1u, m = nb >= 256 ? nb / 256 : (nb >= 16 ? nb / 16 : 1u);
    const uint32_t nwaves = vwin * wpw;
    hipLaunchKernelGGL(k_wsum_q1<typename CV::suite>, dim3((nwaves + 3) / 4), b256, 0, stream, ws.buckets.as(), nb, m, wpw, nwaves, ws.rc.as());
    hipLaunchKernelGGL(k_wsum_q2<typename CV::suite>, dim3(vwin), dim3(64), 0, stream, ws.rc.as(), wpw, ws.bits.as());
    HIP_CHECK(hipMemcpyAsync(rec.bits_host.p, ws.bits.p, (size_t)vwin * 3 * acc_bytes, hipMemcpyDeviceToHost, stream));
    rec.wsum_lg = 4; while ((1u << rec.wsum_lg) < 16 * m) rec.wsum_lg++;
    finish();
    return -(int)vwin;
  }
  if (!ws.owns(rec)) throw HipFailure{hipErrorInvalidValue, __FILE__, __LINE__};
  const int h = (p.c - 1) / 2;
  const uint32_t tasks = (1u << h) + ((uint32_t)p.nb >> h);
  const int nbits = (int)vwin * p.c;
  if constexpr (CV::FIXED_TABLE) if (table_c) {
    uint32_t wps = 1;
    const uint32_t wps_max = batch <= msm_env().wsum_blk_max ? 4 : 1;
    while (wps < wps_max && (uint32_t)p.nb >= 64 * wps * 2) wps *= 2;
    if (wps > 1) {
      hipLaunchKernelGGL(k_wsum_blk<RV>, dim3((unsigned)batch), dim3(64 * wps), (size_t)wps * 2 * acc_bytes, stream, ws.buckets.as(),
                         (uint32_t)p.nb, ws.rc.as());
    } else {
      uint32_t lps_log = 6;
      while (lps_log > 2 && (batch << (lps_log - 1)) >= 2048 * 64) lps_log--;
      while ((1u << lps_log) > (uint32_t)p.nb) lps_log--;
      hipLaunchKernelGGL(k_wsum<RV>, dim3((unsigned)(((batch << lps_log) + 255) / 256)), b256, 0, stream, ws.buckets.as(), (uint32_t)p.nb,
                         (uint32_t)batch, lps_log, ws.rc.as());
    }
    HIP_CHECK(hipMemcpyAsync(rec.bits_host.p, ws.rc.p, batch * (size_t)RV::OUT_WORDS * 4, hipMemcpyDeviceToHost, stream));
    finish();
    return p.c;
  }
  if (p.nb <= 256 && batch >= 8) {
    hipLaunchKernelGGL(k_bits_direct<CV>, dim3(((unsigned)nbits + 127) / 128), dim3(128), 0, stream, ws.buckets.as(), p.c, (uint32_t)nbits, ws.bits.as());
  } else {
    hipLaunchKernelGGL(k_rowcol<CV>, dim3(((size_t)vwin * tasks * 64 + 255) / 256), b256, 0, stream, ws.buckets.as(), p.c, h,
                       vwin * tasks, ws.rc.as());
    hipLaunchKernelGGL(k_bits<CV>, dim3(((size_t)nbits * 64 + 255) / 256), b256, 0, stream, ws.buckets.as(), ws.rc.as(),
                       p.c, h, (uint32_t)nbits, ws.bits.as());
  }
  if (batch >= 8) {
    hipLaunchKernelGGL(k_horner<CV>, dim3(((unsigned)batch + 63) / 64), dim3(64), 0, stream, ws.bits.as(), (uint32_t)(p.nwin * p.c),
                       (uint32_t)batch, ws.rc.as());
    HIP_CHECK(hipMemcpyAsync(rec.bits_host.p, ws.rc.p, batch * acc_bytes, hipMemcpyDeviceToHost, stream));
  } else {
    HIP_CHECK(hipMemcpyAsync(rec.bits_host.p, ws.bits.p, (size_t)nbits * acc_bytes, hipMemcpyDeviceToHost, stream));
  }
  finish();
  return p.nwin * p.c;
}

template <class S>
static int msm_te_enqueue_impl(const te_pre_raw *d_pre, const uint32_t *d_scalars, size_t n, MsmWorkspace &ws, MsmChain &rec, hipStream_t stream) {
  rec.n = n; rec.ret = 0; rec.armed = true;
  MsmLaunch o; o.defer = true;
  if (n) rec.ret = msm_device<TeCurve<S>>((const uint32_t *)d_pre, d_scalars, n, S::Fr::BITS, ws, rec, stream, o);
  return 0;
}
template <class S>
static int msm_te_finish_impl(MsmWorkspace &ws, MsmChain &rec, hipStream_t stream, HostExt *out) {
  using HT = HostTe<S>;
  *out = HT::identity();
  if (!rec.armed) return -1;
  rec.disarm();
  if (rec.n == 0) return 0;
  msm_collect(ws, rec, stream);
  const int nbits = rec.ret, c = rec.plan.c, lg = rec.wsum_lg; const uint32_t *bh = rec.bits_host.as();
  HostExt acc = HT::identity();
  if (nbits < 0) {
    for (int w = -nbits - 1; w >= 0; w--) {
      for (int k = 0; k < c - lg; k++) acc = HT::dbl(acc);
      acc = HT::add(acc, HT::from_raw32(bh + ((size_t)w * 3 + 2) * 32));
      for (int k = 0; k < lg - 4; k++) acc = HT::dbl(acc);
      acc = HT::add(acc, HT::from_raw32(bh + ((size_t)w * 3 + 1) * 32));
      for (int k = 0; k < 4; k++) acc = HT::dbl(acc);
      acc = HT::add(acc, HT::from_raw32(bh + (size_t)w * 3 * 32));
    }
  } else for (int i = nbits - 1; i >= 0; i--) {
    acc = HT::dbl(acc);
    acc = HT::add(acc, HT::from_raw32(bh + (size_t)i * 32));
  }
  *out = acc;
  return 0;
}

int msm_te_enqueue(int suite, const te_pre_raw *d_pre, const uint32_t *d_scalars, size_t n, MsmWorkspace &ws, MsmChain &rec, hipStream_t stream) {
  if (suite < 0 || suite >= AVRF_N_SUITES) return -1;
  return with_suite(suite, [&](auto tag) { using S = typename decltype(tag)::type; return msm_te_enqueue_impl<S>(d_pre, d_scalars, n, ws, rec, stream); });
}
int msm_te_finish(int suite, MsmWorkspace &ws, MsmChain &rec, hipStream_t stream, HostExt *out) {
  if (suite < 0 || suite >= AVRF_N_SUITES) return -1;
  return with_suite(suite, [&](auto tag) { using S = typename decltype(tag)::type; return msm_te_finish_impl<S>(ws, rec, stream, out); });
}
template <class S>
// ... 518 lines not shown
```

### ark_vrf_amd/csrc/pool.hip

```cpp
#include "capi_internal.h"
#include "suite_dispatch.h"
#include "host_sha512.h"
#include "host_sha512_mb.h"
#include "host_numa.h"
#include <pthread.h>
#include <atomic>
#include <condition_variable>
#include <mutex>
#include <string.h>
#include <thread>
#include <time.h>

using namespace avrf;

namespace {

enum SlotState { S_FREE = 0, S_SUBMITTED, S_BEGUN, S_READY, S_HASHED, S_MSM, S_DONE };

struct Slot {
  avrf_ctx *c = nullptr;
  std::atomic<int> state{S_FREE};
  bool has_batch = false;
  bool wire = false; int validate = 0;
  bool from_host = false;
// ... 49 lines not shown
    cyc_issued++;
    return true;
  }
};

namespace {

void scalar_digest(const uint8_t *msg, size_t len, uint8_t out[64]) { HostSha512 h; h.update(msg, len); h.final(out); }

struct Run {
  avrf_pool *P; Worker &W; uint64_t seq = 0;
  Run(avrf_pool *p, Worker &w) : P(p), W(w) {}

  void done(Slot &S, int status) {
    if (S.lane) { S.lane->queued--; S.lane = nullptr; }
    S.c->run_phase = 0; S.c->L = &S.c->own; S.c->stream = nullptr;
    std::lock_guard<std::mutex> lk(P->m);
    if (P->cycling) {
      P->cyc_done++; P->cyc_t_last = now_us();
      if (status != P->cyc_expect) P->cyc_mismatch++;
      S.status = status;
      if (status == P->cyc_expect && P->take_locked()) { S.from_host = P->cyc_from_host; S.state = S_SUBMITTED; }
      else S.state = S_FREE;
    } else { S.status = status; S.state = S_DONE; }
    P->cv_done.notify_all();
  }
  static void latch(Slot &S, int status) { if (S.wire && status == AVRF_INVALID_DATA) S.resident_invalid = true; }

  void begin(Slot &S) {
    const double t0 = thread_cpu_us();
    avrf_ctx *c = S.c;
    c->stream = W.ingest;
    c->L = &c->own;
    int st = AVRF_OK;
    if (!S.from_host && S.resident_invalid) { W.cpu_us[0] += thread_cpu_us() - t0; done(S, AVRF_INVALID_DATA); return; }
    if (S.from_host) {
      S.resident_invalid = false;
      if (S.wire) st = guarded([&] { return ctx_stage_wire(c, P->kind, S.n, S.pks, S.ios, S.io_counts, S.ads, S.ad_lens, S.proofs, S.validate, false); });
      else st = guarded([&] { return ctx_stage(c, P->kind, S.n, nullptr, S.pks, S.ios, S.io_counts, S.ads, S.ad_lens, S.proofs, false); });
      S.has_batch = st == AVRF_OK;
    }
    if (st == AVRF_OK) st = guarded([&] { return batch_begin(c, P->kind); });
    if (st == AVRF_OK && hipEventRecord(S.ev, c->stream) != hipSuccess) { (void)hipGetLastError(); st = AVRF_ERR_NO_DEVICE; }
    W.cpu_us[0] += thread_cpu_us() - t0;
    if (st != AVRF_OK) { done(S, st); return; }
    S.seq = ++seq; S.state = S_BEGUN;
  }

  void hash(std::vector<int> &ready, size_t count) {
    const double t0 = thread_cpu_us();
    WeightJob jobs[16]; WeightJob *pj[16]; Slot *ss[16]; int k = 0;
    for (size_t i = 0; i < count; i++) {
      Slot &S = P->slots[ready[i]];
      if (batch_host_weights(S.c) || S.c->n == 0) {
        int st = guarded([&] { return batch_seed(S.c, P->kind, S.digest); });
        if (st != AVRF_OK) { done(S, st); continue; }
        S.state = S_HASHED;
        continue;
      }
      jobs[k].prefix = nullptr; jobs[k].prefix_len = 0; jobs[k].c16 = nullptr; jobs[k].resp = nullptr; jobs[k].n = 0; jobs[k].rsz = 0;
      jobs[k].msg = S.c->h_msg.as<uint8_t>(); jobs[k].msg_len = S.c->h_msg_len; pj[k] = &jobs[k]; ss[k] = &S; k++;
    }
    if (k == 1 || (k > 1 && !sha512_mb_available())) { for (int i = 0; i < k; i++) scalar_digest(jobs[i].msg, jobs[i].msg_len, jobs[i].digest); }
    else if (k > 1) { if (sha512_mb16_available()) sha512_weights_x16(pj, k); else { sha512_weights_x8(pj, k < 8 ? k : 8); if (k > 8) sha512_weights_x8(pj + 8, k - 8); } }
    for (int i = 0; i < k; i++) { memcpy(ss[i]->digest, jobs[i].digest, 64); ss[i]->state = S_HASHED; }
    ready.erase(ready.begin(), ready.begin() + count);
    if (k) { W.hash_groups++; W.hash_msgs += k; }
    W.cpu_us[2] += thread_cpu_us() - t0;
  }

  Lane *pick_lane() {
    Lane *best = nullptr;
    for (Lane *L : W.lanes) if (L->queued < P->depth && (!best || L->queued < best->queued)) best = L;
    return best;
  }

  void launch(Slot &S) {
    const double t0 = thread_cpu_us();
    S.lane = pick_lane(); S.lane->queued++;
    S.c->L = S.lane; S.c->stream = S.lane->stream;
    int st = guarded([&] { return batch_launch(S.c, P->kind, S.digest); });
    if (st == AVRF_OK && hipEventRecord(S.ev, S.lane->stream) != hipSuccess) { (void)hipGetLastError(); st = AVRF_ERR_NO_DEVICE; }
    W.cpu_us[3] += thread_cpu_us() - t0;
    if (st != AVRF_OK) { if (S.c->run_phase == 2) { (void)hipStreamSynchronize(S.lane->stream); S.c->chain().disarm(); } done(S, st); return; }
    S.seq = ++seq; S.state = S_MSM;
  }

  void finish(Slot &S) {
    const double t0 = thread_cpu_us();
    const int st = guarded([&] { return batch_end(S.c, P->kind); });
    W.cpu_us[4] += thread_cpu_us() - t0;
    done(S, st);
  }

  void loop() {
    (void)hipSetDevice(P->device);
    std::vector<int> ready;
    const double cpu0 = thread_cpu_us();
    for (;;) {
      bool progress = false;
      {
        std::lock_guard<std::mutex> lk(P->m);
        if (P->stop) break;
      }
      size_t n_begun = 0, n_msm = 0;
      Slot *oldest = nullptr;
      for (int si : W.slots) {
        Slot &S = P->slots[si];
        if (S.state != S_MSM) continue;
        if (hipEventQuery(S.ev) == hipSuccess) { finish(S); progress = true; }
        else { (void)hipGetLastError(); n_msm++; if (!oldest || S.seq < oldest->seq) oldest = &S; }
      }
      for (int si : W.slots) {
        Slot &S = P->slots[si];
        if (S.state == S_HASHED && pick_lane()) { launch(S); progress = true; if (S.state == S_MSM) n_msm++; }
      }
      for (int si : W.slots) {
        Slot &S = P->slots[si];
        if (S.state == S_SUBMITTED) { begin(S); progress = true; }
      }
      for (int si : W.slots) {
        Slot &S = P->slots[si];
        if (S.state != S_BEGUN) continue;
        if (hipEventQuery(S.ev) == hipSuccess) {
          const double t0 = thread_cpu_us();
          const int st = guarded([&] { return batch_collect(S.c, P->kind); });
          W.cpu_us[1] += thread_cpu_us() - t0;
          if (st != AVRF_OK) { latch(S, st); done(S, st); } else { S.state = S_READY; ready.push_back(si); }
          progress = true;
        } else { (void)hipGetLastError(); n_begun++; if (!oldest || S.seq < oldest->seq) oldest = &S; }
      }
      if (!ready.empty()) {
        const size_t g = (size_t)P->group;
        if (ready.size() >= g || (n_begun == 0 && 2 * n_msm <= W.capacity)) { hash(ready, ready.size() < g ? ready.size() : g); progress = true; }
      }
      if (progress) continue;
      if (oldest) { W.waits++; (void)hipEventSynchronize(oldest->ev); continue; }
      std::unique_lock<std::mutex> lk(P->m);
      P->cv_work.wait(lk, [&] {
        if (P->stop) return true;
        for (int si : W.slots) if (P->slots[si].state == S_SUBMITTED) return true;
        return false;
      });
    }
    W.cpu_us[5] = thread_cpu_us() - cpu0;
  }
};

}

extern "C" {

int avrf_pool_create(int suite, int device, int kind, int n_slots, int n_lanes, int lane_depth, int n_threads, int hash_group, avrf_pool **out) {
  if (!out || suite < 0 || suite >= AVRF_N_SUITES || (kind != 1 && kind != 2) || n_slots < 1 || n_slots > 4096 || n_lanes < 1 || n_lanes > 64 ||
      lane_depth < 0 || lane_depth > 64 || n_threads < 1 || n_threads > 64 || hash_group < 0 || hash_group > 16) return AVRF_ERR_BAD_ARG;
  *out = nullptr;
  if (n_threads > n_slots) n_threads = n_slots;
  if (n_lanes > n_slots) n_lanes = n_slots;
  if (n_lanes < n_threads) n_lanes = n_threads;
  int nd = 0;
  if (hipGetDeviceCount(&nd) != hipSuccess || device < 0 || device >= nd) return AVRF_ERR_NO_DEVICE;
  HIP_TRY(hipSetDevice(device));
  avrf_pool *P = new avrf_pool();
  P->suite = suite; P->device = device; P->kind = kind;
  P->group = hash_group ? hash_group : 1;
  P->depth = lane_depth ? lane_depth : 3;
  const bool ext = msm_te_pending_supported(suite);
// ... 200 lines not shown
```

### ark_vrf_amd/csrc/te_quad.h

```cpp
#pragma once
#include "te.h"
#include "curves.h"

namespace avrf {

template <int P0, int P1, int P2, int P3> AVRF_DI fp qperm(const fp &a) {
  fp r;
#pragma unroll
  for (int i = 0; i < 8; i++) r.v[i] = (uint32_t)__builtin_amdgcn_mov_dpp((int)a.v[i], P0 | (P1 << 2) | (P2 << 4) | (P3 << 6), 0xf, 0xf, true);
  return r;
}
AVRF_DI fp fp_sel(bool c, const fp &a, const fp &b) {
  fp r;
#pragma unroll
  for (int i = 0; i < 8; i++) r.v[i] = c ? a.v[i] : b.v[i];
  return r;
}
template <class S> AVRF_DI fp q_identity(uint32_t j) { return (j & 1) ? fp_one<typename S::Fq>() : fp_zero(); }

template <class S> __device__ __noinline__ static fp q_add(fp a, fp b, uint32_t j) {
  using Fq = typename S::Fq;
  const fp m1 = fp_mul<Fq>(a, b);
  const fp sa = fp_add<Fq>(a, qperm<1, 0, 3, 2>(a)), sb = fp_add<Fq>(b, qperm<1, 0, 3, 2>(b));
  const bool l2 = j == 2;
  const fp m2 = fp_mul<Fq>(fp_sel(l2, m1, sa), fp_sel(l2, fp_const<Fq>(S::D), sb));
  const fp A = qperm<0, 0, 0, 0>(m1), B = qperm<1, 1, 1, 1>(m1), D = qperm<3, 3, 3, 3>(m1);
  const fp C = qperm<2, 2, 2, 2>(m2), Ep = qperm<0, 0, 0, 0>(m2);
  const fp AB = fp_add<Fq>(A, B), aA = mul_a<S>(A), nC = fp_neg<Fq>(C);
  const fp X = fp_sel(j == 0, Ep, fp_sel(j == 1, B, D));
  const fp Y = fp_sel(j == 0, AB, fp_sel(j == 1, aA, fp_sel(l2, nC, C)));
  const fp U = fp_sub<Fq>(X, Y);
  return fp_mul<Fq>(qperm<0, 1, 0, 3>(U), qperm<3, 2, 1, 2>(U));
}

template <class S> __device__ __noinline__ static fp q_dbl(fp a, uint32_t j) {
  using Fq = typename S::Fq;
  const fp sa = fp_add<Fq>(a, qperm<1, 0, 3, 2>(a));
  const fp m1 = fp_sqr<Fq>(fp_sel(j == 2, qperm<0, 1, 0, 3>(sa), a));
  const fp A = qperm<0, 0, 0, 0>(m1), B = qperm<1, 1, 1, 1>(m1), Sq = qperm<2, 2, 2, 2>(m1), ZZ = qperm<3, 3, 3, 3>(m1);
  const fp aA = mul_a<S>(A);
  const fp X = fp_sel(j == 0, Sq, fp_sel(j == 1, aA, fp_add<Fq>(aA, B)));
  const fp Y = fp_sel(j == 0, fp_add<Fq>(A, B), fp_sel(j == 1, B, fp_sel(j == 2, fp_zero(), fp_add<Fq>(ZZ, ZZ))));
  const fp U = fp_sub<Fq>(X, Y);
  return fp_mul<Fq>(qperm<0, 1, 0, 3>(U), qperm<3, 2, 1, 2>(U));
}

template <class S> __device__ __noinline__ static fp q_madd(fp a, fp x2, fp y2, fp k2, uint32_t j) {
  using Fq = typename S::Fq;
  const fp sa = fp_add<Fq>(a, qperm<1, 0, 3, 2>(a));
  const fp opa = fp_sel(j == 3, qperm<0, 1, 2, 0>(sa), a);
  const fp opb = fp_sel(j == 0, x2, fp_sel(j == 1, y2, fp_sel(j == 2, k2, fp_add<Fq>(x2, y2))));
  const fp m1 = fp_mul<Fq>(opa, opb);
  const fp A = qperm<0, 0, 0, 0>(m1), B = qperm<1, 1, 1, 1>(m1), C = qperm<2, 2, 2, 2>(m1), Ep = qperm<3, 3, 3, 3>(m1), Z1 = qperm<3, 3, 3, 3>(a);
  const fp X = fp_sel(j == 0, Ep, fp_sel(j == 1, B, Z1));
  const fp Y = fp_sel(j == 0, fp_add<Fq>(A, B), fp_sel(j == 1, mul_a<S>(A), fp_sel(j == 2, fp_neg<Fq>(C), C)));
  const fp U = fp_sub<Fq>(X, Y);
  return fp_mul<Fq>(qperm<0, 1, 0, 3>(U), qperm<3, 2, 1, 2>(U));
}

template <class S, int NBITS> __device__ static fp q_smul(const fp &base, const fp &k, uint32_t j) {
  constexpr int NW = (NBITS + 2) / 3, W = (3 * NW + 31) / 32, SH = 32 * W - 3 * NW;
  static_assert(W <= 8 && SH < 32, "scalar window layout");
  fp tab[8];
  tab[0] = q_identity<S>(j); tab[1] = base; tab[2] = q_dbl<S>(base, j);
#pragma unroll 1
  for (int i = 3; i < 8; i++) tab[i] = q_add<S>(tab[i - 1], base, j);
  uint32_t kk[W];
#pragma unroll
  for (int i = W - 1; i >= 0; i--) {
    const uint32_t hi = i < 8 ? k.v[i] : 0u, lo = i >= 1 ? k.v[i - 1] : 0u;
    kk[i] = SH ? (hi << SH) | (lo >> (32 - SH)) : hi;
  }
  fp acc = q_identity<S>(j);
#pragma unroll 1
  for (int w = 0; w < NW; w++) {
    const uint32_t d = kk[W - 1] >> 29;
#pragma unroll
    for (int i = W - 1; i >= 1; i--) kk[i] = (kk[i] << 3) | (kk[i - 1] >> 29);
    kk[0] <<= 3;
    if (w) { acc = q_dbl<S>(acc, j); acc = q_dbl<S>(acc, j); acc = q_dbl<S>(acc, j); }
    fp e = tab[0];
#pragma unroll
    for (uint32_t i = 1; i < 8; i++) e = fp_sel(d == i, tab[i], e);
    acc = q_add<S>(acc, e, j);
  }
// ... 42 lines not shown
    Y.v[i] = j == 0 ? A.v[i] + B.v[i] : (j == 1 ? y1 : (l2 ? -C.v[i] : C.v[i]));
  }
  fu<L> U = fu_carry<Fq>(fu_sub<L>(X, Y));
  if (S::A_KIND == 1) {
    uint32_t h[L - 1];
#pragma unroll
    for (int i = 0; i < L - 1; i++) h[i] = (uint32_t)B.v[i] + 5u * (uint32_t)A.v[i];
    U = fu_sel<L>(j == 1, fu_carry_u<Fq>(h, B.v[L - 1] + 5 * A.v[L - 1]), U);
  }
  return fu_mul<Fq>(fu_qperm<0, 1, 0, 3>(U), fu_qperm<3, 2, 1, 2>(U));
}

template <class S> struct QuadSat {
  using el = fp;
  static AVRF_DI el identity(uint32_t j) { return q_identity<S>(j); }
  static AVRF_DI el add(const el &a, const el &b, uint32_t j) { return q_add<S>(a, b, j); }
  static AVRF_DI el sel(bool c, const el &a, const el &b) { return fp_sel(c, a, b); }
  static AVRF_DI el shfl_down(const el &a, int d) { return fp_shfl_down(a, d); }
  static AVRF_DI el shfl_xor(const el &a, int m) { return fp_shfl_xor(a, m); }
  static AVRF_DI el load(const uint32_t *p) { return load_fp(p); }
  static AVRF_DI void store(uint32_t *p, const el &v) { store_fp(p, v); }
  static AVRF_DI el load_part(const uint32_t *part, size_t k, int j) {
    if constexpr (TeCurve<S>::accum::PART_WORDS == 32) return load_fp(part + k * 32 + j * 8);
    else return teu_load_part_coord<S>(part + k * TEU_PART_WORDS, j);
  }
};
template <class S> struct QuadUns {
  using Fq = typename S::Fq;
  static constexpr int L = UL<Fq>::L;
  using el = fu<L>;
  static AVRF_DI el identity(uint32_t j) { return (j & 1) ? fu_const<Fq>(UL<Fq>::ONE) : fu_zero<L>(); }
  static AVRF_DI el add(const el &a, const el &b, uint32_t j) { return qu_add<S>(a, b, j); }
  static AVRF_DI el sel(bool c, const el &a, const el &b) { return fu_sel<L>(c, a, b); }
  static AVRF_DI el shfl_down(const el &a, int d) { el r;
#pragma unroll
    for (int i = 0; i < L; i++) r.v[i] = __shfl_down(a.v[i], d);
    return r; }
  static AVRF_DI el shfl_xor(const el &a, int m) { el r;
#pragma unroll
    for (int i = 0; i < L; i++) r.v[i] = __shfl_xor(a.v[i], m);
    return r; }
  static AVRF_DI el load(const uint32_t *p) { const fp v = load_fp(p); return fu_slice<Fq, 0>(v.v); }
  static AVRF_DI void store(uint32_t *p, const el &v) { fp r; fu_to_packed<Fq>(r.v, v); store_fp(p, r); }
  static AVRF_DI el load_part(const uint32_t *part, size_t k, int j) { return teu_load_part_coord_raw<S>(part + k * TEU_PART_WORDS, j); }
};
#if !defined(AVRF_NO_UNSAT) && !defined(AVRF_NO_UNSAT_QUAD)
template <class S> using Quad = std::conditional_t<FuAsm<typename S::Fq>::value && !S::SW_NATIVE, QuadUns<S>, QuadSat<S>>;
#else
template <class S> using Quad = QuadSat<S>;
#endif

template <class S> AVRF_DI typename Quad<S>::el q_wave_sum(typename Quad<S>::el v, uint32_t q, uint32_t j) {
  using Q = Quad<S>;
#pragma unroll 1
  for (int off = 8; off >= 1; off >>= 1) {
    const typename Q::el o = Q::shfl_down(v, 4 * off);
    if ((int)q < off) v = Q::add(v, o, j);
  }
  return v;
}
template <class S> AVRF_DI typename Quad<S>::el q_wave_sum2(const typename Quad<S>::el &a, const typename Quad<S>::el &b, uint32_t q, uint32_t j) {
  using Q = Quad<S>;
  const bool lowq = q < 8;
  const typename Q::el send = Q::sel(lowq, b, a);
  const typename Q::el got = Q::shfl_xor(send, 32);
  typename Q::el v = Q::add(Q::sel(lowq, a, b), got, j);
#pragma unroll 1
  for (int off = 4; off >= 1; off >>= 1) {
    const typename Q::el o = Q::shfl_down(v, 4 * off);
    if ((int)(q & 7) < off) v = Q::add(v, o, j);
  }
  return v;
}
template <class S> AVRF_DI typename Quad<S>::el q_wave_suffix(typename Quad<S>::el v, uint32_t q, uint32_t j) {
  using Q = Quad<S>;
#pragma unroll 1
  for (int off = 1; off < 16; off <<= 1) {
    const typename Q::el o = Q::shfl_down(v, 4 * off);
    if ((int)q + off < 16) v = Q::add(v, o, j);
  }
  return v;
}

template <class S>
__global__ void __launch_bounds__(256)
k_wsum_q1(const uint32_t *__restrict__ buckets, uint32_t nb, uint32_t m, uint32_t wpw, uint32_t nwaves, uint32_t *__restrict__ out) {
  const uint32_t gw = (blockIdx.x * blockDim.x + threadIdx.x) >> 6, lane = threadIdx.x & 63, q = lane >> 2, j = lane & 3;
  if (gw >= nwaves) return;
  const uint32_t v = gw / wpw, wi = gw - v * wpw;
  using Q = Quad<S>; using el = typename Q::el;
  const uint32_t *B = buckets + (size_t)v * nb * 32;
  el Sx = Q::identity(j), J = Q::identity(j);
#pragma unroll 1
  for (int k = (int)m - 1; k >= 0; k--) {
    const uint32_t b0 = wi * 16 * m + q + 16 * (uint32_t)k;
    if (b0 < nb) Sx = Q::add(Sx, Q::load(B + (size_t)b0 * 32 + j * 8), j);
    if (k > 0) J = Q::add(J, Sx, j);
  }
  const el A = q_wave_suffix<S>(Sx, q, j);
  const el V = q_wave_sum2<S>(A, J, q, j);
  uint32_t *o = out + (size_t)gw * 3 * 32 + j * 8;
  if (q == 0) { Q::store(o, V); Q::store(o + 64, A); }
  if (q == 8) Q::store(o + 32, V);
}

template <class S>
__global__ void __launch_bounds__(64)
k_wsum_q2(const uint32_t *__restrict__ trip, uint32_t wpw, uint32_t *__restrict__ out) {
  const uint32_t v = blockIdx.x, lane = threadIdx.x & 63, q = lane >> 2, j = lane & 3;
  using Q = Quad<S>; using el = typename Q::el;
  el v1 = Q::identity(j), v2 = v1, y = v1;
  if (q < wpw) {
    const uint32_t *t = trip + ((size_t)v * wpw + q) * 3 * 32 + j * 8;
    v1 = Q::load(t); v2 = Q::load(t + 32); y = Q::load(t + 64);
  }
  const el P12 = q_wave_sum2<S>(v1, v2, q, j);
  el A = q_wave_suffix<S>(y, q, j);
  if (q == 0) A = Q::identity(j);
  const el P3 = q_wave_sum<S>(A, q, j);
  uint32_t *o = out + (size_t)v * 3 * 32 + j * 8;
  if (q == 0) { Q::store(o, P12); Q::store(o + 64, P3); }
  if (q == 8) Q::store(o + 32, P12);
}

template <class S> AVRF_DI void q_heavy_sum(const uint32_t *__restrict__ part, size_t p0, uint32_t np, uint32_t *__restrict__ dst, uint32_t *lds) {
  const uint32_t t = threadIdx.x, lane = t & 63, q = lane >> 2, j = lane & 3, gq = t >> 2, wv = t >> 6;
  using Q = Quad<S>; using el = typename Q::el;
  el a = Q::identity(j);
#pragma unroll 1
  for (uint32_t k = gq; k < np; k += 64) a = Q::add(a, Q::load_part(part, p0 + k, (int)j), j);
  a = q_wave_sum<S>(a, q, j);
  if (q == 0) Q::store(lds + wv * 32 + j * 8, a);
  __syncthreads();
  if (t < 4) {
#pragma unroll 1
    for (uint32_t w = 1; w < 4; w++) a = Q::add(a, Q::load(lds + w * 32 + j * 8), j);
    Q::store(dst + j * 8, a);
  }
  __syncthreads();
}

}
```

### ark_vrf_amd/csrc/vrf_batch.hip

```cpp
#include "vrf_batch.h"
#include "proto_dev.h"
#include "suite_dispatch.h"

#ifndef AVRF_TU_SUITE
#error "vrf_batch.hip is built once per suite: -DAVRF_TU_SUITE=<id> (csrc/Makefile)"
#endif
namespace avrf {

template <class S>
__global__ void __launch_bounds__(128)
k_thin_prepare(BatchDev b, uint32_t *__restrict__ c_out, uint32_t *__restrict__ z_out, uint32_t *__restrict__ flags) {
  using Fr = typename S::Fr;
  uint32_t j = blockIdx.x * blockDim.x + threadIdx.x;
  if (j >= b.n) return;
  uint32_t io0 = b.io_off[j], io1 = b.io_off[j + 1], m = io1 - io0;
  uint32_t ad0 = b.ad_off[j], adl = b.ad_off[j + 1] - ad0;
  uint32_t f = 0;
  suite_tr<S> h; tr_init(h);
  for (int i = 0; i < S::SUITE_ID_LEN; i++) tr_byte(h, S::SUITE_ID[i]);
  tr_byte(h, DS_THIN);
  tr_u64le(h, (uint64_t)m + 1);
  absorb_generator<S>(h);
  sw_enc enc[4]; bool have_enc = false;
  if constexpr (S::SW_CODEC) if (m == 1) {
    const uint8_t *p = b.ios_xy + 128 * (size_t)io0, *pr = b.proofs + 96 * (size_t)j, *pk = b.pks_xy + 64 * (size_t)j;
    const fp xs[4] = {fp_load_le(pk), fp_load_le(p), fp_load_le(p + 64), fp_load_le(pr)};
    const fp ys[4] = {fp_load_le(pk + 32), fp_load_le(p + 32), fp_load_le(p + 96), fp_load_le(pr + 32)};
    sw_encode_te_many<S, 4>(xs, ys, enc); have_enc = true;
  }
  {
    fp x = fp_load_le(b.pks_xy + 64 * (size_t)j), y = fp_load_le(b.pks_xy + 64 * (size_t)j + 32);
    f |= point_flags<S>(x, y);
    if (have_enc) absorb_sw_enc(h, enc[0]); else absorb_point_xy<S>(h, x, y);
  }
  for (uint32_t i = 0; i < m; i++) {
    const uint8_t *p = b.ios_xy + 128 * (size_t)(io0 + i);
    fp x = fp_load_le(p), y = fp_load_le(p + 32);
    f |= point_flags<S>(x, y); if (have_enc) absorb_sw_enc(h, enc[1]); else absorb_point_xy<S>(h, x, y);
    x = fp_load_le(p + 64); y = fp_load_le(p + 96);
    f |= point_flags<S>(x, y); if (have_enc) absorb_sw_enc(h, enc[2]); else absorb_point_xy<S>(h, x, y);
  }
  tr_u64le(h, (uint64_t)adl);
  tr_bytes(h, b.ads + ad0, adl);
  if (m) {
    auto rd = delin_seed(h);
    for (uint32_t i = 0; i < m; i++) {
      uint32_t w[4]; rd_chunk16(rd, i, w);
      uint4 *o = reinterpret_cast<uint4 *>(z_out + 4 * (size_t)(io0 + i));
      *o = make_uint4(w[0], w[1], w[2], w[3]);
    }
  }
  {
    const uint8_t *pr = b.proofs + 96 * (size_t)j;
    fp x = fp_load_le(pr), y = fp_load_le(pr + 32), s = fp_load_le(pr + 64);
    if (point_flags<S>(x, y) & FLAG_RANGE) f |= FLAG_RANGE;
    if (ge_p<Fr>(s)) f |= FLAG_SCALAR;
    tr_byte(h, DS_CHALLENGE);
    if (have_enc) absorb_sw_enc(h, enc[3]); else absorb_point_xy<S>(h, x, y);
    auto rd = tr_reader(h);
    uint32_t w[4]; rd_chunk16(rd, 0, w);
    uint4 *o = reinterpret_cast<uint4 *>(c_out + 4 * (size_t)j);
    *o = make_uint4(w[0], w[1], w[2], w[3]);
    if (b.records) {
      uint4 *r = reinterpret_cast<uint4 *>(b.records + 64 * (size_t)j);
      const uint4 *sp = reinterpret_cast<const uint4 *>(pr + 64);
      r[0] = make_uint4(w[0], w[1], w[2], w[3]); r[1] = make_uint4(0, 0, 0, 0); r[2] = sp[0]; r[3] = sp[1];
    }
  }
  if (f) atomicOr(flags, f);
}

AVRF_DI fp fp_from_u128(const uint32_t *w) {
  fp a = fp_zero(); uint4 v = *reinterpret_cast<const uint4 *>(w);
  a.v[0] = v.x; a.v[1] = v.y; a.v[2] = v.z; a.v[3] = v.w; return a;
}
template <class S> AVRF_DI void emit_term(uint32_t *scalars, te_pre *pre, uint32_t t, const fp &scalar_plain, const uint8_t *xy) {
  using Fq = typename S::Fq;
  store_fp(scalars + 8 * (size_t)t, scalar_plain);
  fp x = fp_to_mont<Fq>(fp_load_le(xy)), y = fp_to_mont<Fq>(fp_load_le(xy + 32));
  store_pre(pre + t, te_make_pre<S>(x, y));
}

template <class S>
__global__ void __launch_bounds__(128)
k_thin_terms(BatchDev b, Seed64 seed, uint64_t j0, const uint32_t *__restrict__ c_in, const uint32_t *__restrict__ z_in,
             uint32_t *__restrict__ scalars, te_pre *__restrict__ pre, uint32_t *__restrict__ gpart) {
  using Fr = typename S::Fr;
  __shared__ fp red[128];
  uint32_t j = blockIdx.x * blockDim.x + threadIdx.x;
  fp ws = fp_zero();
  if (j < b.n) {
    uint32_t io0 = b.io_off[j], m = b.io_off[j + 1] - io0;
    uint64_t gj = j0 + j;
    uint32_t ww[4];
    if (b.weights) { const uint4 v = *reinterpret_cast<const uint4 *>(b.weights + 16 * (size_t)j); ww[0] = v.x; ww[1] = v.y; ww[2] = v.z; ww[3] = v.w; }
    else { uint64_t blk[8]; sha512_xof_block(seed.w, gj >> 2, blk); digest_le128(blk, (int)(gj & 3), ww); }
    fp w_plain = fp_zero(); w_plain.v[0] = ww[0]; w_plain.v[1] = ww[1]; w_plain.v[2] = ww[2]; w_plain.v[3] = ww[3];
    fp w = fp_to_mont<Fr>(w_plain);
    fp c = fp_to_mont<Fr>(fp_from_u128(c_in + 4 * (size_t)j));
    const uint8_t *pr = b.proofs + 96 * (size_t)j;
    fp s = fp_to_mont<Fr>(fp_load_le(pr + 64));
    fp wc = fp_mul<Fr>(w, c);
    ws = fp_mul<Fr>(w, s);
    uint32_t t = 2 * j + 2 * io0;
    emit_term<S>(scalars, pre, t, w_plain, pr);
    emit_term<S>(scalars, pre, t + 1, fp_from_mont<Fr>(wc), b.pks_xy + 64 * (size_t)j);
    for (uint32_t i = 0; i < m; i++) {
      fp z = fp_to_mont<Fr>(fp_from_u128(z_in + 4 * (size_t)(io0 + i)));
      const uint8_t *p = b.ios_xy + 128 * (size_t)(io0 + i);
      emit_term<S>(scalars, pre, t + 2 + 2 * i, fp_from_mont<Fr>(fp_mul<Fr>(wc, z)), p + 64);
      emit_term<S>(scalars, pre, t + 3 + 2 * i, fp_from_mont<Fr>(fp_neg<Fr>(fp_mul<Fr>(ws, z))), p);
    }
  }
  red[threadIdx.x] = ws;
  __syncthreads();
  for (int s2 = 64; s2 >= 1; s2 >>= 1) {
    if ((int)threadIdx.x < s2) red[threadIdx.x] = fp_add<Fr>(red[threadIdx.x], red[threadIdx.x + s2]);
    __syncthreads();
  }
  if (threadIdx.x == 0) store_fp(gpart + 8 * (size_t)blockIdx.x, red[0]);
}

template <class S>
__global__ void __launch_bounds__(256)
k_g_final(const uint32_t *__restrict__ gpart, uint32_t nparts, uint32_t *__restrict__ scalars, te_pre *__restrict__ pre,
          uint32_t t_last, int which_base) {
  using Fr = typename S::Fr; using Fq = typename S::Fq;
  __shared__ fp red[256];
  fp acc = fp_zero();
  for (uint32_t i = threadIdx.x; i < nparts; i += 256) acc = fp_add<Fr>(acc, load_fp(gpart + 8 * (size_t)i));
  red[threadIdx.x] = acc;
  __syncthreads();
  for (int s2 = 128; s2 >= 1; s2 >>= 1) {
    if ((int)threadIdx.x < s2) red[threadIdx.x] = fp_add<Fr>(red[threadIdx.x], red[threadIdx.x + s2]);
    __syncthreads();
  }
  if (threadIdx.x == 0) {
    store_fp(scalars + 8 * (size_t)t_last, fp_from_mont<Fr>(fp_neg<Fr>(red[0])));
    te_pre g;
    if (which_base == 0) { g.x = fp_const<Fq>(S::G_X); g.y = fp_const<Fq>(S::G_Y); g.k = fp_const<Fq>(S::G_K); }
    else { g.x = fp_const<Fq>(S::B_X); g.y = fp_const<Fq>(S::B_Y); g.k = fp_const<Fq>(S::B_K); }
    store_pre(pre + t_last, g);
  }
}



template <class S>
__global__ void __launch_bounds__(128)
k_ped_prepare(BatchDev b, uint32_t *__restrict__ c_out, uint8_t *__restrict__ merged_xy, uint32_t *__restrict__ flags) {
  using Fr = typename S::Fr;
  uint32_t j = blockIdx.x * blockDim.x + threadIdx.x;
  if (j >= b.n) return;
  uint32_t io0 = b.io_off[j], m = b.io_off[j + 1] - io0, ad0 = b.ad_off[j], adl = b.ad_off[j + 1] - ad0;
  const uint8_t *ios = b.ios_xy + 128 * (size_t)io0, *pr = b.proofs + 256 * (size_t)j;
  suite_tr<S> t; uint32_t f = 0;
  tr_base<S>(t, DS_PEDERSEN, false, nullptr, ios, m, b.ads + ad0, adl, &f);
  uint8_t *mo = merged_xy + 128 * (size_t)j;
  if (m == 1) {
    const uint4 *src = reinterpret_cast<const uint4 *>(ios); uint4 *dst = reinterpret_cast<uint4 *>(mo);
#pragma unroll
    for (int i = 0; i < 8; i++) dst[i] = src[i];
  } else if (m == 0) {
    fp zero = fp_zero(), one = fp_zero(); one.v[0] = S::SW_NATIVE ? 0 : 1;
    fp_store_le(mo, zero); fp_store_le(mo + 32, one); fp_store_le(mo + 64, zero); fp_store_le(mo + 96, one);
  } else {
    auto dseed = delin_seed(t);
    te_ext im = te_identity<S>(), om = te_identity<S>();
    for (uint32_t i = 0; i < m; i++) {
      te_pre pi = pre_from_xy<S>(ios + 128 * (size_t)i), po = pre_from_xy<S>(ios + 128 * (size_t)i + 64);
      if (i == 0) { im = te_madd<S>(im, pi); om = te_madd<S>(om, po); }
      else { fp z = xof128(dseed, i - 1); im = te_add<S>(im, te_smul<S>(pi, z, 128)); om = te_add<S>(om, te_smul<S>(po, z, 128)); }
    }
    te_aff ia = te_to_aff<S>(im), oa = te_to_aff<S>(om);
    store_xy<S>(mo, ia); store_xy<S>(mo + 64, oa);
  }
  fp ybx = fp_load_le(pr), yby = fp_load_le(pr + 32), rx = fp_load_le(pr + 64), ry = fp_load_le(pr + 96);
  fp okx = fp_load_le(pr + 128), oky = fp_load_le(pr + 160);
  f |= point_flags<S>(ybx, yby);
  f |= (point_flags<S>(rx, ry) | point_flags<S>(okx, oky)) & FLAG_RANGE;
  if (ge_p<Fr>(fp_load_le(pr + 192)) || ge_p<Fr>(fp_load_le(pr + 224))) f |= FLAG_SCALAR;
  if constexpr (S::SW_CODEC) {
    const fp xs[3] = {ybx, rx, okx}, ys[3] = {yby, ry, oky};
    sw_enc enc[3]; sw_encode_te_many<S, 3>(xs, ys, enc);
    absorb_sw_enc(t, enc[0]); tr_byte(t, DS_CHALLENGE); absorb_sw_enc(t, enc[1]); absorb_sw_enc(t, enc[2]);
  } else {
    absorb_point_xy<S>(t, ybx, yby);
    tr_byte(t, DS_CHALLENGE); absorb_point_xy<S>(t, rx, ry); absorb_point_xy<S>(t, okx, oky);
  }
  fp c = challenge_finish(t);
  *reinterpret_cast<uint4 *>(c_out + 4 * (size_t)j) = make_uint4(c.v[0], c.v[1], c.v[2], c.v[3]);
  if (b.records) {
    uint4 *r = reinterpret_cast<uint4 *>(b.records + 96 * (size_t)j);
    const uint4 *sp = reinterpret_cast<const uint4 *>(pr + 192);
    r[0] = make_uint4(c.v[0], c.v[1], c.v[2], c.v[3]); r[1] = make_uint4(0, 0, 0, 0); r[2] = sp[0]; r[3] = sp[1]; r[4] = sp[2]; r[5] = sp[3];
  }
  if (f) atomicOr(flags, f);
}

template <class S>
__global__ void __launch_bounds__(128)
k_ped_terms(BatchDev b, Seed64 seed, uint64_t j0, const uint32_t *__restrict__ c_in, const uint8_t *__restrict__ merged_xy,
            uint32_t *__restrict__ scalars, te_pre *__restrict__ pre, uint32_t *__restrict__ gpart, uint32_t *__restrict__ bpart) {
  using Fr = typename S::Fr;
  __shared__ fp red[128];
  uint32_t j = blockIdx.x * blockDim.x + threadIdx.x;
  fp us = fp_zero(), usb = fp_zero();
  if (j < b.n) {
    fp t_plain, u_plain;
    if (b.weights) { t_plain = fp_from_u128(reinterpret_cast<const uint32_t *>(b.weights + 32 * (size_t)j)); u_plain = fp_from_u128(reinterpret_cast<const uint32_t *>(b.weights + 32 * (size_t)j + 16)); }
    else {
      ShaReader rd; for (int i = 0; i < 8; i++) rd.seed[i] = seed.w[i]; rd.have = 0;
      t_plain = xof128(rd, (uint32_t)(2 * (j0 + j))); u_plain = xof128(rd, (uint32_t)(2 * (j0 + j) + 1));
    }
    fp tt = fp_to_mont<Fr>(t_plain), uu = fp_to_mont<Fr>(u_plain);
    fp c = fp_to_mont<Fr>(fp_from_u128(c_in + 4 * (size_t)j));
    const uint8_t *pr = b.proofs + 256 * (size_t)j, *mo = merged_xy + 128 * (size_t)j;
    fp s = fp_to_mont<Fr>(fp_load_le(pr + 192)), sb = fp_to_mont<Fr>(fp_load_le(pr + 224));
    uint32_t k = 5 * j;
    emit_term<S>(scalars, pre, k, fp_from_mont<Fr>(fp_mul<Fr>(tt, c)), mo + 64);
    emit_term<S>(scalars, pre, k + 1, t_plain, pr + 128);
    emit_term<S>(scalars, pre, k + 2, fp_from_mont<Fr>(fp_neg<Fr>(fp_mul<Fr>(tt, s))), mo);
    emit_term<S>(scalars, pre, k + 3, fp_from_mont<Fr>(fp_mul<Fr>(uu, c)), pr);
    emit_term<S>(scalars, pre, k + 4, u_plain, pr + 64);
    us = fp_mul<Fr>(uu, s); usb = fp_mul<Fr>(uu, sb);
  }
  red[threadIdx.x] = us;
  __syncthreads();
  for (int s2 = 64; s2 >= 1; s2 >>= 1) {
    if ((int)threadIdx.x < s2) red[threadIdx.x] = fp_add<Fr>(red[threadIdx.x], red[threadIdx.x + s2]);
    __syncthreads();
  }
  if (threadIdx.x == 0) store_fp(gpart + 8 * (size_t)blockIdx.x, red[0]);
  __syncthreads();
  red[threadIdx.x] = usb;
  __syncthreads();
  for (int s2 = 64; s2 >= 1; s2 >>= 1) {
    if ((int)threadIdx.x < s2) red[threadIdx.x] = fp_add<Fr>(red[threadIdx.x], red[threadIdx.x + s2]);
    __syncthreads();
  }
  if (threadIdx.x == 0) store_fp(bpart + 8 * (size_t)blockIdx.x, red[0]);
}

template <class S> void BatchOps<S>::ped_prepare(const BatchDev &b, uint32_t *d_c, uint8_t *d_merged, uint32_t *d_flags, hipStream_t st) {
  if (!b.n) return;
  dim3 g((b.n + 127) / 128), blk(128);
  hipLaunchKernelGGL(k_ped_prepare<S>, g, blk, 0, st, b, d_c, d_merged, d_flags);
}
template <class S> void BatchOps<S>::ped_terms(const BatchDev &b, const Seed64 &seed, uint64_t j0, const uint32_t *d_c, const uint8_t *d_merged,
                                               uint32_t *d_scalars, te_pre_raw *d_pre, uint32_t *d_gpart, uint32_t n_terms, hipStream_t st) {
  if (!b.n) return;
  dim3 g((b.n + 127) / 128), blk(128);
  uint32_t *bp = d_gpart + 8 * (size_t)g.x;
  hipLaunchKernelGGL(k_ped_terms<S>, g, blk, 0, st, b, seed, j0, d_c, d_merged, d_scalars, (te_pre *)d_pre, d_gpart, bp);
  hipLaunchKernelGGL(k_g_final<S>, dim3(1), dim3(256), 0, st, d_gpart, g.x, d_scalars, (te_pre *)d_pre, n_terms - 2, 0);
  hipLaunchKernelGGL(k_g_final<S>, dim3(1), dim3(256), 0, st, bp, g.x, d_scalars, (te_pre *)d_pre, n_terms - 1, 1);
}
template <class S> void BatchOps<S>::thin_prepare(const BatchDev &b, uint32_t *d_c, uint32_t *d_z, uint32_t *d_flags, hipStream_t st) {
  if (!b.n) return;
  dim3 g((b.n + 127) / 128), blk(128);
  hipLaunchKernelGGL(k_thin_prepare<S>, g, blk, 0, st, b, d_c, d_z, d_flags);
}
template <class S> void BatchOps<S>::thin_terms(const BatchDev &b, const Seed64 &seed, uint64_t j0, const uint32_t *d_c, const uint32_t *d_z,
                                                uint32_t *d_scalars, te_pre_raw *d_pre, uint32_t *d_gpart, uint32_t n_terms, hipStream_t st) {
  if (!b.n) return;
  dim3 g((b.n + 127) / 128), blk(128);
  hipLaunchKernelGGL(k_thin_terms<S>, g, blk, 0, st, b, seed, j0, d_c, d_z, d_scalars, (te_pre *)d_pre, d_gpart);
  hipLaunchKernelGGL(k_g_final<S>, dim3(1), dim3(256), 0, st, d_gpart, g.x, d_scalars, (te_pre *)d_pre, n_terms - 1, 0);
}
template struct BatchOps<suite_by_id<AVRF_TU_SUITE>::type>;

}
```

Before: 132.2 million.

## Fuse follow-up reduction and scan kernels via last-block ticket handoff

Adds a last-arriving-workgroup primitive built on an atomic ticket counter and uses it to fold follow-on single-block kernels into their producers. The thin and Pedersen terms kernels now finish the global reduction themselves, the three scan/plan kernels merge into one k_scan, heavy-bucket detection moves into scatter so bucket_sum handles heavy slots in extra blocks, and the two window-sum levels fuse. The goal is to cut kernel launch and inter-kernel drain overhead in the MSM pipeline. In exchange it needs persistent zeroed ticket buffers, extra fences, and reset logic on error paths, and a stale ticket could corrupt later runs.

```diff
diff --git a/ark_vrf_amd/csrc/capi.hip b/ark_vrf_amd/csrc/capi.hip
--- a/ark_vrf_amd/csrc/capi.hip
+++ b/ark_vrf_amd/csrc/capi.hip
@@ -262,7 +262,7 @@
     c->n_terms = kind == 1 ? 2 * n + 2 * c->tot_io + 1 : 5 * n + 2;
     HIP_TRY(c->d_c.ensure(n * 16)); HIP_TRY(c->h_c.ensure(n * 16));
     HIP_TRY(c->d_z.ensure(kind == 1 ? c->tot_io * 16 + 16 : n * 128));
-    if (c->lane_owner) { HIP_TRY(c->L->d_scalars.ensure(c->n_terms * 32)); HIP_TRY(c->L->d_pre.ensure(c->n_terms * sizeof(te_pre_raw))); HIP_TRY(c->L->d_gpart.ensure(((n + 127) / 128) * 64 + 64)); }
+    if (c->lane_owner) { HIP_TRY(c->L->d_scalars.ensure(c->n_terms * 32)); HIP_TRY(c->L->d_pre.ensure(c->n_terms * sizeof(te_pre_raw))); HIP_TRY(ensure_gpart(*c->L, n, c->stream)); }
   }
   if (wait) HIP_TRY(hipStreamSynchronize(c->stream));
   c->staged_kind = kind;
@@ -314,7 +314,7 @@
   c->n_terms = kind == 1 ? 2 * n + 2 * c->tot_io + 1 : 5 * n + 2;
   HIP_TRY(c->d_c.ensure(n * 16)); HIP_TRY(c->h_c.ensure(n * 16));
   HIP_TRY(c->d_z.ensure(kind == 1 ? c->tot_io * 16 + 16 : n * 128));
-  if (c->lane_owner) { HIP_TRY(c->L->d_scalars.ensure(c->n_terms * 32)); HIP_TRY(c->L->d_pre.ensure(c->n_terms * sizeof(te_pre_raw))); HIP_TRY(c->L->d_gpart.ensure(((n + 127) / 128) * 64 + 64)); }
+  if (c->lane_owner) { HIP_TRY(c->L->d_scalars.ensure(c->n_terms * 32)); HIP_TRY(c->L->d_pre.ensure(c->n_terms * sizeof(te_pre_raw))); HIP_TRY(ensure_gpart(*c->L, n, c->stream)); }
   if (!wait) { c->wire_pending = true; c->staged_kind = kind; return AVRF_OK; }
   HIP_TRY(hipStreamSynchronize(c->stream)); HIP_TRY(hipGetLastError());
   if (*h_flag) return AVRF_INVALID_DATA;
@@ -501,7 +501,7 @@
   }
   Seed64 seed;
   for (int i = 0; i < 8; i++) { uint64_t v; memcpy(&v, digest + 8 * i, 8); seed.w[i] = __builtin_bswap64(v); }
-  HIP_TRY(c->L->d_scalars.ensure(c->n_terms * 32)); HIP_TRY(c->L->d_pre.ensure(c->n_terms * sizeof(te_pre_raw))); HIP_TRY(c->L->d_gpart.ensure(((n + 127) / 128) * 64 + 64));
+  HIP_TRY(c->L->d_scalars.ensure(c->n_terms * 32)); HIP_TRY(c->L->d_pre.ensure(c->n_terms * sizeof(te_pre_raw))); HIP_TRY(ensure_gpart(*c->L, n, c->stream));
   const double t2 = now_us();
   if (kind == 1) AVRF_BATCH(c->suite, thin_terms(b, seed, 0, c->d_c.as<uint32_t>(), c->d_z.as<uint32_t>(), c->L->d_scalars.as<uint32_t>(),
                                                  c->L->d_pre.as<te_pre_raw>(), c->L->d_gpart.as<uint32_t>(), (uint32_t)c->n_terms, c->stream));
@@ -559,7 +559,7 @@
 static int run_call(avrf_ctx *c, int (*phase)(avrf_ctx *, int)) {
   if (!c) return AVRF_ERR_BAD_ARG;
   if (!c->staged_kind) {
-    if (c->run_phase) { (void)hipSetDevice(c->device); (void)hipStreamSynchronize(c->stream); c->run_phase = 0; c->chain().disarm(); }
+    if (c->run_phase) { (void)hipSetDevice(c->device); (void)hipStreamSynchronize(c->stream); c->run_phase = 0; c->chain().disarm(); c->L->zero_tickets(c->stream); }
     return AVRF_ERR_BAD_ARG;
   }
   return phase(c, c->staged_kind);
@@ -839,7 +839,7 @@
   c->run_phase = 0;
   if (st != AVRF_OK) return st;
   const size_t nt = c->n_terms;
-  HIP_TRY(c->L->d_scalars.ensure(2 * nt * 32)); HIP_TRY(c->L->d_pre.ensure(nt * sizeof(te_pre_raw))); HIP_TRY(c->L->d_gpart.ensure(2 * 64 + 64));
+  HIP_TRY(c->L->d_scalars.ensure(2 * nt * 32)); HIP_TRY(c->L->d_pre.ensure(nt * sizeof(te_pre_raw))); HIP_TRY(ensure_gpart(*c->L, 2, c->stream));
   c->h_weights.assign(64, 0); c->h_weights[0] = 1; c->h_weights[32 + 16] = 1;
   HIP_TRY(c->d_weights.ensure(64));
   HIP_TRY(hipMemcpyAsync(c->d_weights.p, c->h_weights.data(), 64, hipMemcpyHostToDevice, c->stream));
diff --git a/ark_vrf_amd/csrc/capi_internal.h b/ark_vrf_amd/csrc/capi_internal.h
--- a/ark_vrf_amd/csrc/capi_internal.h
+++ b/ark_vrf_amd/csrc/capi_internal.h
@@ -37,7 +37,17 @@
   int queued = 0;
   MsmWorkspace ws;
   DevBuf d_scalars, d_pre, d_gpart;
+  void zero_tickets(hipStream_t st) {
+    ws.zero_tickets(st);
+    if (d_gpart.p && (hipMemsetAsync(d_gpart.p, 0, 64, st) != hipSuccess || hipStreamSynchronize(st) != hipSuccess)) (void)hipGetLastError();
+  }
 };
+inline hipError_t ensure_gpart(Lane &L, size_t n_items, hipStream_t st) {
+  const size_t bytes = 64 + ((n_items + 127) / 128) * 64;
+  if (bytes <= L.d_gpart.cap && L.d_gpart.p) return hipSuccess;
+  if (hipError_t e = L.d_gpart.ensure(bytes)) return e;
+  return hipMemsetAsync(L.d_gpart.p, 0, 64, st);
+}
 
 }
 
diff --git a/ark_vrf_amd/csrc/handoff.h b/ark_vrf_amd/csrc/handoff.h
--- /dev/null
+++ b/ark_vrf_amd/csrc/handoff.h
@@ -0,0 +1,28 @@
+#pragma once
+#include <hip/hip_runtime.h>
+#include <stdint.h>
+
+namespace avrf {
+
+__device__ __forceinline__ bool wg_last_arriver(uint32_t *counter, uint32_t total, uint32_t *word) {
+  asm volatile("s_waitcnt vmcnt(0)" ::: "memory");
+  __syncthreads();
+  if (threadIdx.x == 0) {
+    __builtin_amdgcn_fence(__ATOMIC_RELEASE, "agent");
+    asm volatile("s_waitcnt vmcnt(0)" ::: "memory");
+    const uint32_t ticket = __hip_atomic_fetch_add(counter, 1u, __ATOMIC_RELAXED, __HIP_MEMORY_SCOPE_AGENT);
+    const uint32_t last = ticket + 1u == total ? 1u : 0u;
+    if (last) {
+      __hip_atomic_store(counter, 0u, __ATOMIC_RELAXED, __HIP_MEMORY_SCOPE_AGENT);
+      __builtin_amdgcn_fence(__ATOMIC_ACQUIRE, "agent");
+      asm volatile("s_waitcnt vmcnt(0)" ::: "memory");
+    }
+    *(volatile uint32_t *)word = last;
+  }
+  __syncthreads();
+  const bool last = *(volatile uint32_t *)word != 0;
+  __syncthreads();
+  return last;
+}
+
+}
diff --git a/ark_vrf_amd/csrc/msm.h b/ark_vrf_amd/csrc/msm.h
--- a/ark_vrf_amd/csrc/msm.h
+++ b/ark_vrf_amd/csrc/msm.h
@@ -56,6 +56,8 @@
 
 struct MsmChain {
   PinMem bits_host, plan_host;
+  static constexpr size_t NO_PLAN_OFF = ~(size_t)0;
+  size_t plan_off = NO_PLAN_OFF;
   DevEvent ev0, ev1;
   MsmPlan plan = {0, 0, 0, 0}; int ret = 0;
   int wsum_lg = 4;
@@ -76,6 +78,7 @@
   DevMem lane_base;
   DevMem heavy;
   DevMem plan_dev;
+  DevMem tickets;
   DevMem buckets;
   DevMem rc;
   DevMem part;
@@ -85,6 +88,8 @@
   double accum_ms_total = 0; uint64_t accum_launches = 0; float accum_ms_last = 0;
   MsmPlan last_plan = {0, 0, 0, 0};
   void ensure(size_t n, const MsmPlan &p, size_t acc_bytes, size_t batch, size_t lanes_max, size_t part_bytes = 0);
+  void ensure_tickets(size_t vwin, hipStream_t stream);
+  void zero_tickets(hipStream_t stream);
   void release() { *this = MsmWorkspace(); }
 };
 
diff --git a/ark_vrf_amd/csrc/msm.hip b/ark_vrf_amd/csrc/msm.hip
--- a/ark_vrf_amd/csrc/msm.hip
+++ b/ark_vrf_amd/csrc/msm.hip
@@ -2,6 +2,7 @@
 #include "host_pool.h"
 #include "curves.h"
 #include "suite_dispatch.h"
+#include "handoff.h"
 #include "te_quad.h"
 #include "host_g1.h"
 #include <stdio.h>
@@ -107,90 +108,93 @@
 }
 
 __global__ void __launch_bounds__(256)
-k_scan_tiles(uint32_t *__restrict__ H, uint32_t ntiles, int c, uint32_t *__restrict__ cnts) {
-  const uint32_t nb = 1u << (c - 1), w = blockIdx.y, b = blockIdx.x * 256 + threadIdx.x;
-  if (b >= nb) return;
-  uint32_t *Hb = H + (size_t)w * ntiles * nb + b;
-  uint32_t run = 0, k = 0;
-  for (; k + 8 <= ntiles; k += 8) {
-    uint32_t v[8];
+k_scan(uint32_t *__restrict__ H, uint32_t ntiles, uint32_t n, int c, uint32_t vwin, uint32_t lanes_target, uint32_t per_min, uint32_t *cnts,
+       uint32_t *__restrict__ offs, uint32_t *win_tot, uint32_t *__restrict__ lane_base, uint32_t *__restrict__ plan, uint32_t *tickets) {
+  __shared__ uint32_t sh[257];
+  const uint32_t nb = 1u << (c - 1), w = blockIdx.y, t = threadIdx.x, b = blockIdx.x * 256 + t;
+  if (b < nb) {
+    uint32_t *Hb = H + (size_t)w * ntiles * nb + b;
+    uint32_t run = 0, k = 0;
+    for (; k + 8 <= ntiles; k += 8) {
+      uint32_t v[8];
 #pragma unroll
-    for (int j = 0; j < 8; j++) v[j] = Hb[(size_t)(k + j) * nb];
+      for (int j = 0; j < 8; j++) v[j] = Hb[(size_t)(k + j) * nb];
 #pragma unroll
-    for (int j = 0; j < 8; j++) { Hb[(size_t)(k + j) * nb] = run; run += v[j]; }
-  }
-  for (; k < ntiles; k++) { const uint32_t v = Hb[(size_t)k * nb]; Hb[(size_t)k * nb] = run; run += v; }
-  cnts[(size_t)w * nb + b] = run;
-}
-__global__ void __launch_bounds__(1024)
-k_scan_offs(const uint32_t *__restrict__ cnts, uint32_t n, int c, uint32_t *__restrict__ offs, uint32_t *__restrict__ win_tot) {
-  __shared__ uint32_t part[1024];
-  const uint32_t nb = 1u << (c - 1), w = blockIdx.x, t = threadIdx.x;
-  const uint32_t bpt = (nb + 1023) / 1024;
-  uint32_t b0 = t * bpt, b1 = b0 + bpt; if (b1 > nb) b1 = nb; if (b0 > nb) b0 = nb;
-  uint32_t sum = 0;
-  for (uint32_t b = b0; b < b1; b++) sum += cnts[(size_t)w * nb + b];
-  part[t] = sum;
+      for (int j = 0; j < 8; j++) { Hb[(size_t)(k + j) * nb] = run; run += v[j]; }
+    }
+    for (; k < ntiles; k++) { const uint32_t v = Hb[(size_t)k * nb]; Hb[(size_t)k * nb] = run; run += v; }
+    cnts[(size_t)w * nb + b] = run;
+  }
+  if (!wg_last_arriver(tickets + w, gridDim.x, sh + 256)) return;
+  auto scan256 = [&](uint32_t mine) {
+    sh[t] = mine;
+    __syncthreads();
+    for (uint32_t off = 1; off < 256; off <<= 1) {
+      const uint32_t v = (t >= off) ? sh[t - off] : 0;
+      __syncthreads();
+      sh[t] += v;
+      __syncthreads();
+    }
+  };
+  {
+    const uint32_t bpt = (nb + 255) / 256;
+    uint32_t b0 = t * bpt, b1 = b0 + bpt; if (b1 > nb) b1 = nb; if (b0 > nb) b0 = nb;
+    const uint32_t *cw = cnts + (size_t)w * nb;
+    uint32_t sum = 0;
+    for (uint32_t k = b0; k < b1; k++) sum += cw[k];
+    scan256(sum);
+    if (t == 255) win_tot[w] = sh[255];
+    uint32_t run = sh[t] - sum + w * n;
+    for (uint32_t k = b0; k < b1; k++) { offs[(size_t)w * nb + k] = run; run += cw[k]; }
+  }
+  if (!wg_last_arriver(tickets + vwin, vwin, sh + 256)) return;
+  uint32_t s = 0;
+  for (uint32_t v = t; v < vwin; v += 256) s += win_tot[v];
+  sh[t] = s;
   __syncthreads();
-  for (uint32_t off = 1; off < 1024; off <<= 1) {
-    uint32_t v = (t >= off) ? part[t - off] : 0;
-    __syncthreads();
-    part[t] += v;
-    __syncthreads();
-  }
-  if (t == 1023) win_tot[w] = part[1023];
-  uint32_t run = part[t] - sum + w * n;
-  for (uint32_t b = b0; b < b1; b++) { offs[(size_t)w * nb + b] = run; run += cnts[(size_t)w * nb + b]; }
-}
-
-__global__ void __launch_bounds__(1024)
-k_plan(const uint32_t *__restrict__ win_tot, uint32_t vwin, uint32_t lanes_target, uint32_t per_min, uint32_t *__restrict__ lane_base,
-       uint32_t *__restrict__ plan) {
-  __shared__ uint64_t red[1024];
-  __shared__ uint32_t sc[1024];
-  __shared__ uint32_t carry_s;
-  const uint32_t t = threadIdx.x;
-  uint64_t s = 0;
-  for (uint32_t v = t; v < vwin; v += 1024) s += win_tot[v];
-  red[t] = s;
+  for (uint32_t off = 128; off >= 1; off >>= 1) { if (t < off) sh[t] += sh[t + off]; __syncthreads(); }
+  const uint32_t total = sh[0];
   __syncthreads();
-  for (uint32_t off = 512; off >= 1; off >>= 1) { if (t < off) red[t] += red[t + off]; __syncthreads(); }
-  const uint64_t total = red[0];
   if (lanes_target > 8 * vwin) lanes_target -= vwin;
-  uint64_t per64 = (total + lanes_target - 1) / lanes_target;
+  uint64_t per64 = ((uint64_t)total + lanes_target - 1) / lanes_target;
   if (per64 < per_min) per64 = per_min;
   const uint32_t per = (uint32_t)per64;
-  if (t == 0) carry_s = 0;
-  __syncthreads();
-  for (uint32_t base = 0; base < vwin; base += 1024) {
+  uint32_t carry = 0;
+  for (uint32_t base = 0; base < vwin; base += 256) {
     const uint32_t v = base + t;
     const uint32_t mine = v < vwin ? (win_tot[v] + per - 1) / per : 0;
-    sc[t] = mine;
+    scan256(mine);
+    if (v < vwin) lane_base[v] = carry + sh[t] - mine;
+    carry += sh[255];
     __syncthreads();
-    for (uint32_t off = 1; off < 1024; off <<= 1) {
-      uint32_t x = (t >= off) ? sc[t - off] : 0;
-      __syncthreads();
-      sc[t] += x;
-      __syncthreads();
-    }
-    if (v < vwin) lane_base[v] = carry_s + sc[t] - mine;
-    __syncthreads();
-    if (t == 1023) carry_s += sc[1023];
-    __syncthreads();
-  }
-  if (t == 0) { lane_base[vwin] = carry_s; plan[0] = per; plan[1] = carry_s; plan[2] = 0; }
-}
+  }
+  if (t == 0) { lane_base[vwin] = carry; plan[0] = per; plan[1] = carry; plan[2] = 0; }
+}
+
+constexpr uint32_t HEAVY_PARTIALS = 12;
 
 __global__ void __launch_bounds__(256)
 k_scatter(const uint16_t *__restrict__ keys, uint32_t n, uint32_t tile_len, int c, const uint32_t *__restrict__ H,
           const uint32_t *__restrict__ offs, uint32_t *__restrict__ sorted, uint32_t remap_n, uint32_t remap_stride,
-          const uint32_t *__restrict__ bidx, uint32_t ntiles, uint32_t vwin) {
+          const uint32_t *__restrict__ bidx, uint32_t ntiles, uint32_t vwin, const uint32_t *__restrict__ cnts, uint32_t *__restrict__ plan,
+          uint32_t *__restrict__ heavy) {
   extern __shared__ uint32_t lds[];
   const uint32_t nb = 1u << (c - 1);
   const uint32_t xcd = blockIdx.x & 7u, k = blockIdx.x >> 3, tile = k % ntiles, w = xcd + 8u * (k / ntiles);
   if (w >= vwin) return;
   const uint32_t *Hin = H + ((size_t)w * ntiles + tile) * nb;
-  for (uint32_t b = threadIdx.x; b < nb; b += blockDim.x) lds[b] = offs[(size_t)w * nb + b] + Hin[b];
+  const uint32_t per = plan[0];
+  for (uint32_t b = threadIdx.x; b < nb; b += blockDim.x) {
+    const uint32_t slot = w * nb + b, o = offs[slot];
+    lds[b] = o + Hin[b];
+    if (tile == 0) {
+      const uint32_t cnt = cnts[slot];
+      if ((uint64_t)cnt > (uint64_t)(HEAVY_PARTIALS - 2) * per) {
+        const uint32_t rel = o - w * n, lf = rel / per, ll = (rel + cnt - 1) / per;
+        if (ll - lf + 1 > HEAVY_PARTIALS) heavy[atomicAdd(&plan[2], 1u)] = slot;
+      }
+    }
+  }
   __syncthreads();
   uint32_t lo = tile * tile_len, hi = lo + tile_len; if (hi > n) hi = n;
   const uint16_t *kw = keys + (size_t)w * n;
@@ -294,56 +298,62 @@
 template <class T> struct type_tag { using type = T; };
 template <class CV> AVRF_DI typename CV::acc_t wave_sum(typename CV::acc_t acc);
 
-constexpr uint32_t HEAVY_PARTIALS = 12;
 template <class CV>
 __global__ void __launch_bounds__(256, CV::RED_WAVES)
 k_bucket_sum(const uint32_t *__restrict__ offs, const uint32_t *__restrict__ cnts, const uint32_t *__restrict__ lane_base,
-             uint32_t *__restrict__ plan, uint32_t nslots, uint32_t nb, uint32_t n, const uint32_t *__restrict__ part,
-             uint32_t *__restrict__ buckets, uint32_t *__restrict__ heavy) {
+             const uint32_t *__restrict__ plan, uint32_t nslots, uint32_t nb, uint32_t n, const uint32_t *__restrict__ part,
+             uint32_t *__restrict__ buckets, const uint32_t *__restrict__ heavy, uint32_t own_blocks) {
   using acc_t = typename CV::acc_t;
+  extern __shared__ uint32_t lds[];
+  const uint32_t per = plan[0];
+  if (blockIdx.x >= own_blocks) {
+    const uint32_t nheavy = plan[2], t = threadIdx.x, lane = t & 63, wv = t >> 6;
+    for (uint32_t h = blockIdx.x - own_blocks; h < nheavy; h += gridDim.x - own_blocks) {
+      const uint32_t slot = heavy[h], cnt = cnts[slot];
+      const uint32_t v = slot / nb, rel = offs[slot] - v * n;
+      const uint32_t lf = rel / per, ll = (rel + cnt - 1) / per, np = ll - lf + 1;
+      const size_t p0 = (size_t)lane_base[v] + lf + slot;
+      if constexpr (CV::QUAD) { q_heavy_sum<typename CV::suite>(part, p0, np, buckets + (size_t)slot * CV::ACC_WORDS, lds); continue; }
+      acc_t a = CV::identity();
+#pragma unroll 1
+      for (uint32_t k = t; k < np; k += 256) a = cv_add<CV>(a, CV::accum::load_part(part + (p0 + k) * CV::accum::PART_WORDS));
+      a = wave_sum<CV>(a);
+      if (lane == 0) CV::store_acc(lds + wv * CV::ACC_WORDS, a);
+      __syncthreads();
+      if (t == 0) {
+#pragma unroll 1
+        for (uint32_t w = 1; w < 4; w++) a = cv_add<CV>(a, CV::load_acc(lds + w * CV::ACC_WORDS));
+        CV::store_acc(buckets + (size_t)slot * CV::ACC_WORDS, a);
+      }
+      __syncthreads();
+    }
+    return;
+  }
   const uint32_t slot = blockIdx.x * blockDim.x + threadIdx.x;
   if (slot >= nslots) return;
-  const uint32_t per = plan[0];
   const uint32_t cnt = cnts[slot];
-  if (!cnt) { if (!CV::ZERO_IS_IDENTITY) CV::store_acc(buckets + (size_t)slot * CV::ACC_WORDS, CV::identity()); return; }
+  if (!cnt) {
+    if constexpr (CV::ZERO_IS_IDENTITY) {
+      uint32_t *o = buckets + (size_t)slot * CV::ACC_WORDS;
+      if constexpr (CV::ACC_WORDS % 4 == 0) {
+#pragma unroll
+        for (int i = 0; i < CV::ACC_WORDS / 4; i++) reinterpret_cast<uint4 *>(o)[i] = make_uint4(0, 0, 0, 0);
+      } else {
+#pragma unroll
+        for (int i = 0; i < CV::ACC_WORDS; i++) o[i] = 0;
+      }
+    } else CV::store_acc(buckets + (size_t)slot * CV::ACC_WORDS, CV::identity());
+    return;
+  }
   const uint32_t v = slot / nb, rel = offs[slot] - v * n;
   const uint32_t lf = rel / per, ll = (rel + cnt - 1) / per, np = ll - lf + 1;
-  if (np > HEAVY_PARTIALS) { heavy[atomicAdd(&plan[2], 1u)] = slot; return; }
+  if (np > HEAVY_PARTIALS) return;
   const size_t p0 = (size_t)lane_base[v] + lf + slot;
   using AC = typename CV::accum;
   acc_t acc = AC::load_part(part + p0 * AC::PART_WORDS);
 #pragma unroll 1
   for (uint32_t k = 1; k < np; k++) acc = cv_add<CV>(acc, AC::load_part(part + (p0 + k) * AC::PART_WORDS));
   CV::store_acc(buckets + (size_t)slot * CV::ACC_WORDS, acc);
-}
-
-template <class CV>
-__global__ void __launch_bounds__(256, CV::RED_WAVES)
-k_heavy_sum(const uint32_t *__restrict__ offs, const uint32_t *__restrict__ cnts, const uint32_t *__restrict__ lane_base,
-            const uint32_t *__restrict__ plan, uint32_t nb, uint32_t n, const uint32_t *__restrict__ part,
-            uint32_t *__restrict__ buckets, const uint32_t *__restrict__ heavy) {
-  using acc_t = typename CV::acc_t;
-  extern __shared__ uint32_t lds[];
-  const uint32_t per = plan[0], nheavy = plan[2], t = threadIdx.x, lane = t & 63, wv = t >> 6;
-  for (uint32_t h = blockIdx.x; h < nheavy; h += gridDim.x) {
-    const uint32_t slot = heavy[h], cnt = cnts[slot];
-    const uint32_t v = slot / nb, rel = offs[slot] - v * n;
-    const uint32_t lf = rel / per, ll = (rel + cnt - 1) / per, np = ll - lf + 1;
-    const size_t p0 = (size_t)lane_base[v] + lf + slot;
-    if constexpr (CV::QUAD) { q_heavy_sum<typename CV::suite>(part, p0, np, buckets + (size_t)slot * CV::ACC_WORDS, lds); continue; }
-    acc_t a = CV::identity();
-#pragma unroll 1
-    for (uint32_t k = t; k < np; k += 256) a = cv_add<CV>(a, CV::accum::load_part(part + (p0 + k) * CV::accum::PART_WORDS));
-    a = wave_sum<CV>(a);
-    if (lane == 0) CV::store_acc(lds + wv * CV::ACC_WORDS, a);
-    __syncthreads();
-    if (t == 0) {
-#pragma unroll 1
-      for (uint32_t w = 1; w < 4; w++) a = cv_add<CV>(a, CV::load_acc(lds + w * CV::ACC_WORDS));
-      CV::store_acc(buckets + (size_t)slot * CV::ACC_WORDS, a);
-    }
-    __syncthreads();
-  }
 }
 
 
@@ -600,7 +610,17 @@
   plan_dev.ensure(64);
   ws_buf(buckets, nbk * acc_bytes, 9); ws_buf(rc, nbk * acc_bytes, 10);
   ws_buf(part, (lanes_max + nbk + 64) * (part_bytes ? part_bytes : acc_bytes) + 64, 11);
-  ws_buf(bits, nbits * acc_bytes, 12); own.ensure(nbits * acc_bytes);
+  ws_buf(bits, nbits * acc_bytes + 64, 12); own.ensure(nbits * acc_bytes + 64);
+}
+void MsmWorkspace::ensure_tickets(size_t vwin, hipStream_t stream) {
+  const size_t bytes = (vwin + 2) * 4;
+  if (bytes <= tickets.cap) return;
+  ws_buf(tickets, bytes, 13);
+  HIP_CHECK(hipMemsetAsync(tickets.p, 0, tickets.cap, stream));
+}
+void MsmWorkspace::zero_tickets(hipStream_t stream) {
+  if (!tickets) return;
+  if (hipMemsetAsync(tickets.p, 0, tickets.cap, stream) != hipSuccess || hipStreamSynchronize(stream) != hipSuccess) (void)hipGetLastError();
 }
 
 void MsmChain::ensure(size_t bytes) {
@@ -612,7 +632,7 @@
 static void msm_collect(MsmWorkspace &ws, MsmChain &rec, hipStream_t stream) {
   if (ws.owns(rec)) { HIP_CHECK(hipStreamSynchronize(stream)); HIP_CHECK(hipGetLastError()); }
   HIP_CHECK(hipEventElapsedTime(&ws.accum_ms_last, rec.ev0, rec.ev1));
-  rec.plan.lpb = (int)rec.plan_host.as()[0];
+  rec.plan.lpb = (int)(rec.plan_off != MsmChain::NO_PLAN_OFF ? *(const uint32_t *)(rec.bits_host.as<uint8_t>() + rec.plan_off) : rec.plan_host.as()[0]);
   ws.accum_ms_total += ws.accum_ms_last; ws.accum_launches++; ws.last_plan = rec.plan;
 }
 
@@ -667,7 +687,7 @@
     p.c = 1; p.nwin = scalar_bits; p.nb = 1; p.lpb = 0;
     const size_t acc_b = (size_t)CV::ACC_WORDS * 4, nbits = (size_t)scalar_bits;
     ws.ensure(n_in, p, acc_b, batch, 256);
-    rec.ensure(batch * nbits * acc_b); rec.plan_host.as()[0] = 0; rec.plan = p;
+    rec.ensure(batch * nbits * acc_b); rec.plan_host.as()[0] = 0; rec.plan_off = MsmChain::NO_PLAN_OFF; rec.plan = p;
     HIP_CHECK(hipEventRecord(rec.ev0, stream));
     unsigned threads = 64; while (threads < n_in && threads < 256) threads <<= 1;
     hipLaunchKernelGGL(k_msm_tiny_bits<CV>, dim3((unsigned)nbits, (unsigned)batch), dim3(threads), (threads / 64) * acc_b, stream, d_bases, d_scalars, (uint32_t)n_in,
@@ -701,40 +721,39 @@
   hipLaunchKernelGGL(k_digits, dim3((unsigned)((n_in + 255) / 256), (unsigned)batch), b256, 0, stream, d_scalars, (uint32_t)n_in, (uint32_t)scalar_stride,
                      p.c, dig_nwin, ws.keys.as<uint16_t>(), scalars_mont);
   hipLaunchKernelGGL(k_hist, dim3(ntiles, vwin), b256, lds_bytes, stream, ws.keys.as<uint16_t>(), (uint32_t)n, tile_len, p.c, ws.hist.as());
-  hipLaunchKernelGGL(k_scan_tiles, dim3((unsigned)((p.nb + 255) / 256), vwin), b256, 0, stream, ws.hist.as(), ntiles, p.c, ws.cnts.as());
-  hipLaunchKernelGGL(k_scan_offs, dim3(vwin), dim3(1024), 0, stream, ws.cnts.as(), (uint32_t)n, p.c, ws.offsets.as(), ws.win_tot.as());
-  hipLaunchKernelGGL(k_plan, dim3(1), dim3(1024), 0, stream, ws.win_tot.as(), vwin, (uint32_t)lanes_target, (uint32_t)msm_env().per_min,
-                     ws.lane_base.as(), ws.plan_dev.as());
+  ws.ensure_tickets(vwin, stream);
+  hipLaunchKernelGGL(k_scan, dim3((unsigned)((p.nb + 255) / 256), vwin), b256, 0, stream, ws.hist.as(), ntiles, (uint32_t)n, p.c, vwin, (uint32_t)lanes_target,
+                     (uint32_t)msm_env().per_min, ws.cnts.as(), ws.offsets.as(), ws.win_tot.as(), ws.lane_base.as(), ws.plan_dev.as(), ws.tickets.as());
   hipLaunchKernelGGL(k_scatter, dim3(8u * ((vwin + 7u) / 8u) * ntiles), b256, lds_bytes, stream, ws.keys.as<uint16_t>(), (uint32_t)n, tile_len, p.c, ws.hist.as(),
-                     ws.offsets.as(), ws.sorted.as(), remap_n, remap_stride, d_base_idx, ntiles, vwin);
-  rec.ensure((size_t)vwin * 3 * acc_bytes);
-  if (CV::ZERO_IS_IDENTITY) HIP_CHECK(hipMemsetAsync(ws.buckets.p, 0, (size_t)nbk * acc_bytes, stream));
+                     ws.offsets.as(), ws.sorted.as(), remap_n, remap_stride, d_base_idx, ntiles, vwin, ws.cnts.as(), ws.plan_dev.as(), ws.heavy.as());
+  rec.ensure((size_t)vwin * 3 * acc_bytes + 8);
   HIP_CHECK(hipEventRecord(rec.ev0, stream));
   hipLaunchKernelGGL(k_accumulate<CV>, dim3((unsigned)((lanes_max + 255) / 256)), b256, accumulate_shape<CV>().lds, stream, d_bases, ws.sorted.as(),
                      ws.offsets.as(), ws.win_tot.as(), ws.lane_base.as(), ws.plan_dev.as(), vwin, (uint32_t)p.nb, (uint32_t)n, ws.part.as());
   HIP_CHECK(hipEventRecord(rec.ev1, stream));
   auto bucket_sums = [&](auto tag) {
     using BV = typename decltype(tag)::type;
-    hipLaunchKernelGGL(k_bucket_sum<BV>, dim3((nbk + 255) / 256), b256, 0, stream, ws.offsets.as(), ws.cnts.as(), ws.lane_base.as(), ws.plan_dev.as(), nbk,
-                       (uint32_t)p.nb, (uint32_t)n, ws.part.as(), ws.buckets.as(), ws.heavy.as());
-    hipLaunchKernelGGL(k_heavy_sum<BV>, dim3(nbk < 1024 ? nbk : 1024), b256, 4 * acc_bytes, stream, ws.offsets.as(), ws.cnts.as(), ws.lane_base.as(),
-                       ws.plan_dev.as(), (uint32_t)p.nb, (uint32_t)n, ws.part.as(), ws.buckets.as(), ws.heavy.as());
+    const uint32_t own_blocks = (nbk + 255) / 256;
+    hipLaunchKernelGGL(k_bucket_sum<BV>, dim3(own_blocks + (nbk < 1024 ? nbk : 1024)), b256, 4 * acc_bytes, stream, ws.offsets.as(), ws.cnts.as(), ws.lane_base.as(),
+                       ws.plan_dev.as(), nbk, (uint32_t)p.nb, (uint32_t)n, ws.part.as(), ws.buckets.as(), ws.heavy.as(), own_blocks);
   };
   if (red) bucket_sums(type_tag<RV>{}); else bucket_sums(type_tag<CV>{});
-  HIP_CHECK(hipMemcpyAsync(rec.plan_host.p, ws.plan_dev.p, 8, hipMemcpyDeviceToHost, stream));
   rec.plan = p;
   if constexpr (CV::WINDOW_SUMS) if (batch == 1 && msm_env().window_sums) {
     const uint32_t nb = (uint32_t)p.nb;
     const uint32_t wpw = nb >= 256 ? 16u : 1u, m = nb >= 256 ? nb / 256 : (nb >= 16 ? nb / 16 : 1u);
     const uint32_t nwaves = vwin * wpw;
-    hipLaunchKernelGGL(k_wsum_q1<typename CV::suite>, dim3((nwaves + 3) / 4), b256, 0, stream, ws.buckets.as(), nb, m, wpw, nwaves, ws.rc.as());
-    hipLaunchKernelGGL(k_wsum_q2<typename CV::suite>, dim3(vwin), dim3(64), 0, stream, ws.rc.as(), wpw, ws.bits.as());
-    HIP_CHECK(hipMemcpyAsync(rec.bits_host.p, ws.bits.p, (size_t)vwin * 3 * acc_bytes, hipMemcpyDeviceToHost, stream));
+    hipLaunchKernelGGL(k_wsum_q1<typename CV::suite>, dim3((nwaves + 3) / 4), b256, 0, stream, ws.buckets.as(), nb, m, wpw, nwaves, ws.rc.as(), ws.bits.as(),
+                       ws.tickets.as(), ws.plan_dev.as());
+    rec.plan_off = (size_t)vwin * 3 * acc_bytes;
+    HIP_CHECK(hipMemcpyAsync(rec.bits_host.p, ws.bits.p, (size_t)vwin * 3 * acc_bytes + 8, hipMemcpyDeviceToHost, stream));
     rec.wsum_lg = 4; while ((1u << rec.wsum_lg) < 16 * m) rec.wsum_lg++;
     finish();
     return -(int)vwin;
   }
   if (!ws.owns(rec)) throw HipFailure{hipErrorInvalidValue, __FILE__, __LINE__};
+  rec.plan_off = MsmChain::NO_PLAN_OFF;
+  HIP_CHECK(hipMemcpyAsync(rec.plan_host.p, ws.plan_dev.p, 8, hipMemcpyDeviceToHost, stream));
   const int h = (p.c - 1) / 2;
   const uint32_t tasks = (1u << h) + ((uint32_t)p.nb >> h);
   const int nbits = (int)vwin * p.c;
diff --git a/ark_vrf_amd/csrc/pool.hip b/ark_vrf_amd/csrc/pool.hip
--- a/ark_vrf_amd/csrc/pool.hip
+++ b/ark_vrf_amd/csrc/pool.hip
@@ -155,7 +155,7 @@
     int st = guarded([&] { return batch_launch(S.c, P->kind, S.digest); });
     if (st == AVRF_OK && hipEventRecord(S.ev, S.lane->stream) != hipSuccess) { (void)hipGetLastError(); st = AVRF_ERR_NO_DEVICE; }
     W.cpu_us[3] += thread_cpu_us() - t0;
-    if (st != AVRF_OK) { if (S.c->run_phase == 2) { (void)hipStreamSynchronize(S.lane->stream); S.c->chain().disarm(); } done(S, st); return; }
+    if (st != AVRF_OK) { if (S.c->run_phase == 2) { (void)hipStreamSynchronize(S.lane->stream); S.c->chain().disarm(); S.lane->zero_tickets(S.lane->stream); } done(S, st); return; }
     S.seq = ++seq; S.state = S_MSM;
   }
 
diff --git a/ark_vrf_amd/csrc/te_quad.h b/ark_vrf_amd/csrc/te_quad.h
--- a/ark_vrf_amd/csrc/te_quad.h
+++ b/ark_vrf_amd/csrc/te_quad.h
@@ -1,6 +1,7 @@
 #pragma once
 #include "te.h"
 #include "curves.h"
+#include "handoff.h"
 
 namespace avrf {
 
@@ -209,32 +210,7 @@
   return v;
 }
 
-template <class S>
-__global__ void __launch_bounds__(256)
-k_wsum_q1(const uint32_t *__restrict__ buckets, uint32_t nb, uint32_t m, uint32_t wpw, uint32_t nwaves, uint32_t *__restrict__ out) {
-  const uint32_t gw = (blockIdx.x * blockDim.x + threadIdx.x) >> 6, lane = threadIdx.x & 63, q = lane >> 2, j = lane & 3;
-  if (gw >= nwaves) return;
-  const uint32_t v = gw / wpw, wi = gw - v * wpw;
-  using Q = Quad<S>; using el = typename Q::el;
-  const uint32_t *B = buckets + (size_t)v * nb * 32;
-  el Sx = Q::identity(j), J = Q::identity(j);
-#pragma unroll 1
-  for (int k = (int)m - 1; k >= 0; k--) {
-    const uint32_t b0 = wi * 16 * m + q + 16 * (uint32_t)k;
-    if (b0 < nb) Sx = Q::add(Sx, Q::load(B + (size_t)b0 * 32 + j * 8), j);
-    if (k > 0) J = Q::add(J, Sx, j);
-  }
-  const el A = q_wave_suffix<S>(Sx, q, j);
-  const el V = q_wave_sum2<S>(A, J, q, j);
-  uint32_t *o = out + (size_t)gw * 3 * 32 + j * 8;
-  if (q == 0) { Q::store(o, V); Q::store(o + 64, A); }
-  if (q == 8) Q::store(o + 32, V);
-}
-
-template <class S>
-__global__ void __launch_bounds__(64)
-k_wsum_q2(const uint32_t *__restrict__ trip, uint32_t wpw, uint32_t *__restrict__ out) {
-  const uint32_t v = blockIdx.x, lane = threadIdx.x & 63, q = lane >> 2, j = lane & 3;
+template <class S> AVRF_DI void q_wsum_level2(const uint32_t *trip, uint32_t wpw, uint32_t v, uint32_t *__restrict__ out, uint32_t q, uint32_t j) {
   using Q = Quad<S>; using el = typename Q::el;
   el v1 = Q::identity(j), v2 = v1, y = v1;
   if (q < wpw) {
@@ -250,6 +226,41 @@
   if (q == 8) Q::store(o + 32, P12);
 }
 
+template <class S>
+__global__ void __launch_bounds__(256)
+k_wsum_q1(const uint32_t *__restrict__ buckets, uint32_t nb, uint32_t m, uint32_t wpw, uint32_t nwaves, uint32_t *trip, uint32_t *__restrict__ out,
+          uint32_t *tickets, const uint32_t *__restrict__ plan) {
+  __shared__ uint32_t sh[4];
+  const uint32_t gw = (blockIdx.x * blockDim.x + threadIdx.x) >> 6, lane = threadIdx.x & 63, q = lane >> 2, j = lane & 3;
+  const bool live = gw < nwaves;
+  const uint32_t v = gw / wpw, wi = gw - v * wpw;
+  using Q = Quad<S>; using el = typename Q::el;
+  if (blockIdx.x == 0 && threadIdx.x < 2) out[(size_t)(nwaves / wpw) * 3 * 32 + threadIdx.x] = plan[threadIdx.x];
+  if (live) {
+    const uint32_t *B = buckets + (size_t)v * nb * 32;
+    el Sx = Q::identity(j), J = Q::identity(j);
+#pragma unroll 1
+    for (int k = (int)m - 1; k >= 0; k--) {
+      const uint32_t b0 = wi * 16 * m + q + 16 * (uint32_t)k;
+      if (b0 < nb) Sx = Q::add(Sx, Q::load(B + (size_t)b0 * 32 + j * 8), j);
+      if (k > 0) J = Q::add(J, Sx, j);
+    }
+    const el A = q_wave_suffix<S>(Sx, q, j);
+    const el V = q_wave_sum2<S>(A, J, q, j);
+    uint32_t *o = trip + (size_t)gw * 3 * 32 + j * 8;
+    if (q == 0) { Q::store(o, V); Q::store(o + 64, A); }
+    if (q == 8) Q::store(o + 32, V);
+  }
+  if (wpw >= 4) {
+    if (!wg_last_arriver(tickets + v, wpw / 4, sh)) return;
+    if (threadIdx.x >= 64) return;
+  } else {
+    if (!live) return;
+    asm volatile("s_waitcnt vmcnt(0)" ::: "memory");
+  }
+  q_wsum_level2<S>(trip, wpw, v, out, q, j);
+}
+
 template <class S> AVRF_DI void q_heavy_sum(const uint32_t *__restrict__ part, size_t p0, uint32_t np, uint32_t *__restrict__ dst, uint32_t *lds) {
   const uint32_t t = threadIdx.x, lane = t & 63, q = lane >> 2, j = lane & 3, gq = t >> 2, wv = t >> 6;
   using Q = Quad<S>; using el = typename Q::el;
diff --git a/ark_vrf_amd/csrc/vrf_batch.hip b/ark_vrf_amd/csrc/vrf_batch.hip
--- a/ark_vrf_amd/csrc/vrf_batch.hip
+++ b/ark_vrf_amd/csrc/vrf_batch.hip
@@ -1,5 +1,6 @@
 #include "vrf_batch.h"
 #include "proto_dev.h"
+#include "handoff.h"
 #include "suite_dispatch.h"
 
 #ifndef AVRF_TU_SUITE
@@ -82,11 +83,33 @@
 }
 
 template <class S>
+AVRF_DI void g_final(fp *red, const uint32_t *gpart, uint32_t nparts, uint32_t *__restrict__ scalars, te_pre *__restrict__ pre, uint32_t t_last, int which_base) {
+  using Fr = typename S::Fr; using Fq = typename S::Fq;
+  fp acc = fp_zero();
+  for (uint32_t i = threadIdx.x; i < nparts; i += 128) acc = fp_add<Fr>(acc, load_fp(gpart + 8 * (size_t)i));
+  red[threadIdx.x] = acc;
+  __syncthreads();
+  for (int s2 = 64; s2 >= 1; s2 >>= 1) {
+    if ((int)threadIdx.x < s2) red[threadIdx.x] = fp_add<Fr>(red[threadIdx.x], red[threadIdx.x + s2]);
+    __syncthreads();
+  }
+  if (threadIdx.x == 0) {
+    store_fp(scalars + 8 * (size_t)t_last, fp_from_mont<Fr>(fp_neg<Fr>(red[0])));
+    te_pre g;
+    if (which_base == 0) { g.x = fp_const<Fq>(S::G_X); g.y = fp_const<Fq>(S::G_Y); g.k = fp_const<Fq>(S::G_K); }
+    else { g.x = fp_const<Fq>(S::B_X); g.y = fp_const<Fq>(S::B_Y); g.k = fp_const<Fq>(S::B_K); }
+    store_pre(pre + t_last, g);
+  }
+  __syncthreads();
+}
+
+template <class S>
 __global__ void __launch_bounds__(128)
 k_thin_terms(BatchDev b, Seed64 seed, uint64_t j0, const uint32_t *__restrict__ c_in, const uint32_t *__restrict__ z_in,
-             uint32_t *__restrict__ scalars, te_pre *__restrict__ pre, uint32_t *__restrict__ gpart) {
+             uint32_t *__restrict__ scalars, te_pre *__restrict__ pre, uint32_t *gpart, uint32_t t_last) {
   using Fr = typename S::Fr;
   __shared__ fp red[128];
+  uint32_t *const ticket = gpart; gpart += 16;
   uint32_t j = blockIdx.x * blockDim.x + threadIdx.x;
   fp ws = fp_zero();
   if (j < b.n) {
@@ -119,31 +142,9 @@
     __syncthreads();
   }
   if (threadIdx.x == 0) store_fp(gpart + 8 * (size_t)blockIdx.x, red[0]);
-}
-
-template <class S>
-__global__ void __launch_bounds__(256)
-k_g_final(const uint32_t *__restrict__ gpart, uint32_t nparts, uint32_t *__restrict__ scalars, te_pre *__restrict__ pre,
-          uint32_t t_last, int which_base) {
-  using Fr = typename S::Fr; using Fq = typename S::Fq;
-  __shared__ fp red[256];
-  fp acc = fp_zero();
-  for (uint32_t i = threadIdx.x; i < nparts; i += 256) acc = fp_add<Fr>(acc, load_fp(gpart + 8 * (size_t)i));
-  red[threadIdx.x] = acc;
-  __syncthreads();
-  for (int s2 = 128; s2 >= 1; s2 >>= 1) {
-    if ((int)threadIdx.x < s2) red[threadIdx.x] = fp_add<Fr>(red[threadIdx.x], red[threadIdx.x + s2]);
-    __syncthreads();
-  }
-  if (threadIdx.x == 0) {
-    store_fp(scalars + 8 * (size_t)t_last, fp_from_mont<Fr>(fp_neg<Fr>(red[0])));
-    te_pre g;
-    if (which_base == 0) { g.x = fp_const<Fq>(S::G_X); g.y = fp_const<Fq>(S::G_Y); g.k = fp_const<Fq>(S::G_K); }
-    else { g.x = fp_const<Fq>(S::B_X); g.y = fp_const<Fq>(S::B_Y); g.k = fp_const<Fq>(S::B_K); }
-    store_pre(pre + t_last, g);
-  }
-}
-
+  if (!wg_last_arriver(ticket, gridDim.x, red[1].v)) return;
+  g_final<S>(red, gpart, gridDim.x, scalars, pre, t_last, 0);
+}
 
 
 template <class S>
@@ -201,9 +202,11 @@
 template <class S>
 __global__ void __launch_bounds__(128)
 k_ped_terms(BatchDev b, Seed64 seed, uint64_t j0, const uint32_t *__restrict__ c_in, const uint8_t *__restrict__ merged_xy,
-            uint32_t *__restrict__ scalars, te_pre *__restrict__ pre, uint32_t *__restrict__ gpart, uint32_t *__restrict__ bpart) {
+            uint32_t *__restrict__ scalars, te_pre *__restrict__ pre, uint32_t *gpart, uint32_t t_last) {
   using Fr = typename S::Fr;
   __shared__ fp red[128];
+  uint32_t *const ticket = gpart; gpart += 16;
+  uint32_t *const bpart = gpart + 8 * (size_t)gridDim.x;
   uint32_t j = blockIdx.x * blockDim.x + threadIdx.x;
   fp us = fp_zero(), usb = fp_zero();
   if (j < b.n) {
@@ -240,6 +243,9 @@
     __syncthreads();
   }
   if (threadIdx.x == 0) store_fp(bpart + 8 * (size_t)blockIdx.x, red[0]);
+  if (!wg_last_arriver(ticket, gridDim.x, red[1].v)) return;
+  g_final<S>(red, gpart, gridDim.x, scalars, pre, t_last - 1, 0);
+  g_final<S>(red, bpart, gridDim.x, scalars, pre, t_last, 1);
 }
 
 template <class S> void BatchOps<S>::ped_prepare(const BatchDev &b, uint32_t *d_c, uint8_t *d_merged, uint32_t *d_flags, hipStream_t st) {
@@ -251,10 +257,7 @@
                                                uint32_t *d_scalars, te_pre_raw *d_pre, uint32_t *d_gpart, uint32_t n_terms, hipStream_t st) {
   if (!b.n) return;
   dim3 g((b.n + 127) / 128), blk(128);
-  uint32_t *bp = d_gpart + 8 * (size_t)g.x;
-  hipLaunchKernelGGL(k_ped_terms<S>, g, blk, 0, st, b, seed, j0, d_c, d_merged, d_scalars, (te_pre *)d_pre, d_gpart, bp);
-  hipLaunchKernelGGL(k_g_final<S>, dim3(1), dim3(256), 0, st, d_gpart, g.x, d_scalars, (te_pre *)d_pre, n_terms - 2, 0);
-  hipLaunchKernelGGL(k_g_final<S>, dim3(1), dim3(256), 0, st, bp, g.x, d_scalars, (te_pre *)d_pre, n_terms - 1, 1);
+  hipLaunchKernelGGL(k_ped_terms<S>, g, blk, 0, st, b, seed, j0, d_c, d_merged, d_scalars, (te_pre *)d_pre, d_gpart, n_terms - 1);
 }
 template <class S> void BatchOps<S>::thin_prepare(const BatchDev &b, uint32_t *d_c, uint32_t *d_z, uint32_t *d_flags, hipStream_t st) {
   if (!b.n) return;
@@ -265,8 +268,7 @@
                                                 uint32_t *d_scalars, te_pre_raw *d_pre, uint32_t *d_gpart, uint32_t n_terms, hipStream_t st) {
   if (!b.n) return;
   dim3 g((b.n + 127) / 128), blk(128);
-  hipLaunchKernelGGL(k_thin_terms<S>, g, blk, 0, st, b, seed, j0, d_c, d_z, d_scalars, (te_pre *)d_pre, d_gpart);
-  hipLaunchKernelGGL(k_g_final<S>, dim3(1), dim3(256), 0, st, d_gpart, g.x, d_scalars, (te_pre *)d_pre, n_terms - 1, 0);
+  hipLaunchKernelGGL(k_thin_terms<S>, g, blk, 0, st, b, seed, j0, d_c, d_z, d_scalars, (te_pre *)d_pre, d_gpart, n_terms - 1);
 }
 template struct BatchOps<suite_by_id<AVRF_TU_SUITE>::type>;
 
```

Measured after the change: 128.3 million. -2.9%, worse.
